# oicr-gsi/ConsensusCruncher

Measured on AMD Instinct MI355X. Metric: input reads/sec through SSCS+DCS+SC consensus, higher is better.
Workload: dtype u8

## Files before the change

consensuscruncher_amd/csrc/cc_engine.hip:

```cpp
#include <algorithm>
#include <climits>
#include <cstdint>
#include <cstdio>
#include <cstring>

#include <dlfcn.h>
#include <sched.h>

#include <chrono>

#include <hip/hip_runtime.h>
#include <atomic>
#include <map>
#include <memory>
#include <mutex>
#include <type_traits>
#include <string>
#include <unordered_set>
#include <vector>

#include "../../include/consensuscruncher_amd.h"

static std::atomic<long long> g_launches{0};
#undef hipLaunchKernelGGL
#define hipLaunchKernelGGL(kernelName, ...)                                                          \
    do {                                                                                            \
        g_launches.fetch_add(1, std::memory_order_relaxed);                                         \
        hipLaunchKernelGGLInternal((kernelName), __VA_ARGS__);                                      \
    } while (0)
#define hipMemsetAsync(...) (g_launches.fetch_add(1, std::memory_order_relaxed), ::hipMemsetAsync(__VA_ARGS__))
#define hipMemcpyAsync(...) (g_launches.fetch_add(1, std::memory_order_relaxed), ::hipMemcpyAsync(__VA_ARGS__))

enum : uint32_t {
    EB_COLLISION = 1u << 0,
    EB_DUP_QNAME = 1u << 1,
    EB_AMBIGUOUS = 1u << 2,
    EB_N_HIGHQ = 1u << 3,
    EB_BAD_BASE = 1u << 4,
    EB_SHORT = 1u << 5,
    EB_NO_QUAL = 1u << 6,
    EB_NO_CIGAR = 1u << 7,
    EB_RG = 1u << 8,
    EB_THR = 1u << 9,
    EB_TOO_LONG = 1u << 10,
    EB_KEYERROR = 1u << 12,
    EB_CHAIN = 1u << 13,
    EB_NEEDSORT = 1u << 14,
    EB_PLAN = 1u << 11,
    EB_DEEPSORT = 1u << 15,
    EB_SCANWAIT = 1u << 16,
    EB_GUARD = 1u << 17,
};

__device__ unsigned int g_guard;
__device__ __noinline__ int64_t guard_fail() {
    atomicOr(&g_guard, 1u);
    return 0;
}
#ifdef CC_DEBUG_BOUNDS
__device__ unsigned long long g_dbg_fault;
__device__ __noinline__ int64_t dbg_fail(int site, int64_t i) {
    atomicCAS(&g_dbg_fault, 0ULL, ((unsigned long long)site << 48) | ((unsigned long long)i & 0xffffffffffffULL));
    return 0;
}
__device__ __forceinline__ int64_t dbg_idx(int64_t i, int64_t n, int site) {
    return (i < 0 || i >= n) ? dbg_fail(site, i) : i;
}
#define CC_IDX(i, n, site) ((std::remove_cv_t<std::remove_reference_t<decltype(i)>>)dbg_idx((int64_t)(i), (int64_t)(n), (site)))
#elif defined(CC_NO_GUARD)
#define CC_IDX(i, n, site) (i)
#else
__device__ __forceinline__ int64_t guard_idx(int64_t i, int64_t n) {
    return (uint64_t)i < (uint64_t)n ? i : guard_fail();
}
#define CC_IDX(i, n, site) ((std::remove_cv_t<std::remove_reference_t<decltype(i)>>)guard_idx((int64_t)(i), (int64_t)(n)))
#endif
enum : int {
    DS_REC = 1, DS_QNAME = 2, DS_PAYLOAD = 3, DS_SLOT = 4, DS_PAIR = 5, DS_MEMBER = 6, DS_VOTE_REC = 7,
};

struct TagKey {
    int32_t bc, tid, pos, mtid, mpos, cigA, cigB;
    uint32_t bits;
};
struct CKey {
    int32_t bc, tidLo, posLo, tidHi, posHi, cigA, cigB;
    uint32_t strand;
    uint32_t abstlen;
    uint32_t pad[3];
};

constexpr int GRP_SMALL = 64;

struct alignas(32) RecCore {
    int32_t tid, pos, mtid, mpos, tlen, cig, bc, flag;
};

struct DevTable {
    int64_t n;
    int32_t *tid, *pos, *mtid, *mpos, *tlen, *cig, *qlen, *lseq, *bc, *rg;
    uint16_t* flag;
    uint8_t *mapq, *rflags;
    uint64_t* qn_off;
// ... 340 lines not shown
    for (int i = 4; i < nw; ++i) h = hcomb(h, w[i]);
    return hcomb(h, (uint64_t)len);
}
__device__ __forceinline__ bool qname_eq(const DevTable& T, int32_t a, int32_t b) {
    a = CC_IDX(a, T.n, DS_REC);
    b = CC_IDX(b, T.n, DS_REC);
    const uint64_t oa = T.qn_ol[a], ob = T.qn_ol[b];
    const int la = (int)(oa & 0xffffu), lb = (int)(ob & 0xffffu);
    const uint64_t* wa = reinterpret_cast<const uint64_t*>(T.qn_blob + CC_IDX(oa >> 16, T.qn_bytes + 1, DS_QNAME));
    const uint64_t* wb = reinterpret_cast<const uint64_t*>(T.qn_blob + CC_IDX(ob >> 16, T.qn_bytes + 1, DS_QNAME));
    const int nw = ((la < lb ? la : lb) + 7) >> 3;
    uint64_t d = la != lb ? 1ULL : 0ULL;
#pragma unroll
    for (int i = 0; i < 4; ++i)
        if (i < nw) d |= wa[i] ^ wb[i];
    for (int i = 4; i < nw && !d; ++i) d |= wa[i] ^ wb[i];
    return d == 0;
}

__device__ __forceinline__ int32_t readlane_i32(int32_t v, int k) { return __builtin_amdgcn_readlane(v, k); }
__device__ __forceinline__ uint64_t readlane_u64(uint64_t v, int k) {
    uint32_t lo = (uint32_t)__builtin_amdgcn_readlane((int)(uint32_t)v, k);
    uint32_t hi = (uint32_t)__builtin_amdgcn_readlane((int)(uint32_t)(v >> 32), k);
    return ((uint64_t)hi << 32) | lo;
}

__device__ __forceinline__ int64_t xcd_block() {
    const uint32_t nb = gridDim.x, b = blockIdx.x;
    const uint32_t q = nb >> 3, rem = nb & 7u, x = b & 7u;
    return (int64_t)(x * q + (x < rem ? x : rem) + (b >> 3));
}

__device__ __forceinline__ void wave_add(uint32_t v, uint32_t* dst) {
#pragma unroll
    for (int o = 32; o > 0; o >>= 1) v += __shfl_xor(v, o);
    if ((threadIdx.x & 63) == 0 && v) atomicAdd(dst, v);
}

constexpr int PSTRIPES = 64, PSTRIDE = 16;
__device__ __forceinline__ void stripe_add(uint32_t v, uint32_t* stripes) {
#pragma unroll
    for (int o = 32; o > 0; o >>= 1) v += __shfl_xor(v, o);
    const uint32_t w = blockIdx.x * (blockDim.x >> 6) + (threadIdx.x >> 6);
    if ((threadIdx.x & 63) == 0 && v) atomicAdd(stripes + PSTRIDE * (w & (PSTRIPES - 1)), v);
}

__global__ __launch_bounds__(64) void k_stripe_total(uint32_t* __restrict__ stripes, uint32_t* __restrict__ total) {
    const int t = threadIdx.x;
    uint32_t v = stripes[PSTRIDE * t];
    stripes[PSTRIDE * t] = 0u;
#pragma unroll
    for (int o = 32; o > 0; o >>= 1) v += __shfl_xor(v, o);
    if (t == 0) *total = v;
}

struct FillSet {
    static constexpr int K = 12;
    uint32_t* p[K];
    int64_t n[K];
    uint32_t v[K];
    int k;
};
__global__ __launch_bounds__(256) void k_fill(FillSet fs) {
    const int64_t stride = (int64_t)gridDim.x * blockDim.x;
    const int64_t t = (int64_t)blockIdx.x * blockDim.x + threadIdx.x;
    for (int d = 0; d < fs.k; ++d) {
        uint32_t* p = fs.p[d];
        const int64_t n = fs.n[d];
        const int64_t n4 = ((uintptr_t)p & 15u) ? 0 : n >> 2;
        const uint32_t v = fs.v[d];
        uint4* p4 = reinterpret_cast<uint4*>(p);
        for (int64_t i = t; i < n4; i += stride) p4[i] = make_uint4(v, v, v, v);
        for (int64_t i = 4 * n4 + t; i < n; i += stride) p[i] = v;
    }
}

constexpr int CNT_STRIPES = 64;
__device__ __forceinline__ unsigned long long* cnt_stripe(unsigned long long* cnt) {
    return cnt + CC_NUM_COUNTERS * (blockIdx.x & (CNT_STRIPES - 1));
}

template <int NC>
__device__ __forceinline__ void block_count(int (&v)[NC], const int (&slot)[NC], unsigned long long* cnt) {
    __shared__ int s_red[4][NC];
    const int lane = threadIdx.x & 63, wv = threadIdx.x >> 6;
#pragma unroll
    for (int c = 0; c < NC; ++c) {
        int x = v[c];
        for (int o = 32; o > 0; o >>= 1) x += __shfl_down(x, o);
        if (lane == 0) s_red[wv][c] = x;
    }
    __syncthreads();
#pragma unroll
    for (int c = 0; c < NC; ++c)
        if ((int)threadIdx.x == c) {
            int t = 0;
            for (int w = 0; w < (int)(blockDim.x >> 6); ++w) t += s_red[w][c];
            if (t) atomicAdd(&cnt_stripe(cnt)[slot[c]], (unsigned long long)t);
        }
}


struct ClassifyOut {
    uint64_t* skey;
    uint32_t* sval;
    uint8_t* badflag;
// ... 368 lines not shown
    }
    (void)qkey;
    return m == 1 ? cand : -1;
}

__device__ __forceinline__ int32_t mate_search_global(int64_t N, const uint64_t* __restrict__ rkey,
                                                      const uint64_t* __restrict__ rq, const DevTable& T,
                                                      int32_t r, int32_t mtid, int32_t mpos, uint64_t target,
                                                      uint64_t key, int64_t hint, const uint64_t* __restrict__ gq,
                                                      const int32_t* __restrict__ gend,
                                                      const uint32_t* __restrict__ boff) {
    int64_t x = 0;
    {
        int64_t hi = hint, lo = hint;
        for (int64_t step = 256;; step <<= 2) {
            lo = hi - step;
            if (lo <= 0) { lo = 0; break; }
            if (rkey[lo] < target) break;
            hi = lo;
        }
        x = lo;
        while (x < hi) {
            const int64_t mid = (x + hi) >> 1;
            if (rkey[mid] < target) x = mid + 1;
            else hi = mid;
        }
    }
    if (x + GRP_SMALL + 1 < N && rkey[x] == target && rkey[x + GRP_SMALL + 1] == target)
        return gq ? deep_find(gq, gend, boff, rq, x, key, r) : -1;
    int32_t cand = -1, m = 0, ng = 0;
    for (bool over = false; !over; x += 4) {
        uint64_t kk[4], qq[4];
#pragma unroll
        for (int u = 0; u < 4; ++u) {
            kk[u] = x + u < N ? rkey[x + u] : 0ULL;
            qq[u] = x + u < N ? rq[x + u] : 0ULL;
        }
#pragma unroll
        for (int u = 0; u < 4; ++u) {
            if (over || (x + u < N && kk[u] < target)) continue;
            if (x + u >= N || kk[u] != target) { over = true; continue; }
            if (ng > GRP_SMALL) return -1;
            ++ng;
            if (x + u != r && qq[u] == key) { cand = (int32_t)(x + u); ++m; }
        }
    }
    return m == 1 ? cand : -1;
}

__device__ __forceinline__ bool mate_record(int64_t s, int32_t sx, uint64_t key, int32_t* __restrict__ partner,
                                            int32_t* __restrict__ claimer, int32_t* __restrict__ mate_of,
                                            uint8_t* __restrict__ pflag, unsigned long long* __restrict__ ltab,
                                            uint64_t lmask, uint32_t& n_long, bool both_search,
                                            uint32_t* __restrict__ err) {
    partner[s] = sx;
    claimer[sx] = (int32_t)s;
    const int32_t s1 = (int32_t)s < sx ? (int32_t)s : sx, s2 = (int32_t)s < sx ? sx : (int32_t)s;
    mate_of[s2] = s1;
    pflag[s2] = 1;
    const bool enters = !both_search || s == s2;
    if (ltab && s2 - s1 > PD_W && enters) {
        ++n_long;
        uint64_t h = key & lmask;
        bool done = false;
        for (uint64_t i = 0; i <= lmask && !done; ++i) {
            const unsigned long long prev = atomicCAS(&ltab[h], ~0ULL, key);
            if (prev == ~0ULL) done = true;
            else if (prev == key) { atomicOr(err, EB_NEEDSORT); done = true; }
            else h = (h + 1) & lmask;
        }
        if (!done) atomicOr(err, EB_NEEDSORT);
    } else if (!ltab && s2 - s1 > PD_W && enters) {
        ++n_long;
    }
    return enters;
}

constexpr int PC_HALO = 512;
constexpr int64_t PC_SMALL_N = (int64_t)1 << 23;
template <int TILE>
__global__ __launch_bounds__(256) void k_pair_coord_tile(int64_t N, const uint64_t* __restrict__ skey,
                                                         const int32_t* __restrict__ spos,
                                                         const uint64_t* __restrict__ rkey, DevTable T,
                                                         int32_t* __restrict__ partner, int32_t* __restrict__ claimer,
                                                         int32_t* __restrict__ mate_of, uint8_t* __restrict__ pflag,
                                                         unsigned long long* __restrict__ ltab, uint64_t lmask,
                                                         uint32_t* __restrict__ long_stripes, uint32_t* __restrict__ err,
                                                         const uint64_t* __restrict__ gq, const int32_t* __restrict__ gend,
                                                         const uint32_t* __restrict__ boff,
                                                         const unsigned long long* __restrict__ dgk, uint64_t dgmask,
                                                         uint64_t* __restrict__ pkeys, uint32_t* __restrict__ pcount,
                                                         uint32_t pcap) {
    __shared__ uint64_t s_k[(TILE + PC_HALO + GRP_SMALL + 2)], s_q[(TILE + PC_HALO + GRP_SMALL + 2)];
    const int64_t t0 = xcd_block() * TILE;
    const int64_t t1 = min(N, t0 + TILE);
    const int64_t w0 = t0 > PC_HALO ? t0 - PC_HALO : 0;
    const int64_t w1 = min(N, t1 + GRP_SMALL + 2);
    const int nw = (int)(w1 - w0);
    int32_t mt[TILE / 256], mp[TILE / 256];
#pragma unroll
    for (int u = 0; u < TILE / 256; ++u) {
        const int64_t s = t0 + threadIdx.x + 256 * u;
        mt[u] = s < t1 ? T.mtid[s] : 0;
        mp[u] = s < t1 ? T.mpos[s] : 0;
    }
    for (int i = threadIdx.x; i < nw; i += blockDim.x) {
        s_k[i] = rkey[w0 + i];
        s_q[i] = skey[w0 + i];
    }
    __syncthreads();
    constexpr int PC_PER = TILE / 256;
    int32_t cand[PC_PER];
    uint64_t key[PC_PER], tgt[PC_PER];
#pragma unroll
    for (int u = 0; u < PC_PER; ++u) {
        const int64_t s = t0 + threadIdx.x + 256 * u;
        cand[u] = -1;
        key[u] = ~0ULL;
        tgt[u] = ~0ULL;
        if (s >= t1) continue;
        const int li = (int)(s - w0);
        key[u] = s_q[li];
        if (!spos) partner[s] = -1;
        if (key[u] == ~0ULL) continue;
        const int32_t r = (int32_t)s;
        const int32_t mtid = mt[u], mpos = mp[u];
        const uint64_t target = pos_key(mtid, mpos);
        tgt[u] = target;
        if (target > s_k[li]) continue;
        if (dgk) {
            const int2 dg = dg_lookup(dgk, dgmask, target);
            if (dg.x >= 0) {
                cand[u] = deep_find(gq, gend, boff, skey, dg.x, key[u], r, dg.y);
                continue;
            }
        }
        int lo = 0, hi = li;
        while (lo < hi) {
            const int mid = (lo + hi) >> 1;
            if (s_k[mid] < target) lo = mid + 1;
            else hi = mid;
        }
        if (lo == 0 && w0 > 0) {
            int x = 0;
            while (x < nw && x <= GRP_SMALL + 1 && s_k[x] == target) ++x;
            cand[u] = x > GRP_SMALL + 1 && !gq ? -1
                      : mate_search_global(N, rkey, skey, T, r, mtid, mpos, target, key[u], w0, gq, gend, boff);
        } else {
            int x = lo, ng = 0, m = 0, c = -1;
            bool deep = false;
            for (; x < nw && s_k[x] == target; ++x) {
                if (ng > GRP_SMALL) { deep = true; break; }
                ++ng;
                if (x != li && s_q[x] == key[u]) { c = (int32_t)(w0 + x); ++m; }
            }
            if (deep) c = gq ? deep_find(gq, gend, boff, skey, w0 + lo, key[u], r) : -1;
            else if (x == nw && w1 < N)
                c = mate_search_global(N, rkey, skey, T, r, mtid, mpos, target, key[u], w0 + lo, gq, gend, boff);
            else if (m != 1) c = -1;
            cand[u] = c;
        }
    }
    bool ok[PC_PER];
    {
        int la[PC_PER], lb[PC_PER];
        const uint64_t* wa[PC_PER];
        const uint64_t* wb[PC_PER];
#pragma unroll
        for (int u = 0; u < PC_PER; ++u) {
            const int32_t r = (int32_t)(t0 + threadIdx.x + 256 * u), c = cand[u] < 0 ? r : cand[u];
            const bool f = cand[u] >= 0;
            const uint64_t oa = f ? T.qn_ol[r] : 0ULL, ob = f ? T.qn_ol[c] : 0ULL;
            la[u] = (int)(oa & 0xffffu);
            lb[u] = (int)(ob & 0xffffu);
            wa[u] = reinterpret_cast<const uint64_t*>(T.qn_blob + (oa >> 16));
            wb[u] = reinterpret_cast<const uint64_t*>(T.qn_blob + (ob >> 16));
        }
#pragma unroll
        for (int u = 0; u < PC_PER; ++u) {
            const int nw8 = (la[u] + 7) >> 3;
            uint64_t d = la[u] != lb[u] ? 1ULL : 0ULL;
#pragma unroll
            for (int w = 0; w < 4; ++w)
                if (w < nw8) d |= wa[u][w] ^ wb[u][w];
            for (int w = 4; w < nw8 && !d; ++w) d |= wa[u][w] ^ wb[u][w];
            ok[u] = cand[u] >= 0 && d == 0;
        }
    }
    uint32_t nl = 0, na = 0;
    uint64_t ak[PC_PER];
#pragma unroll
    for (int u = 0; u < PC_PER; ++u) {
        ak[u] = 0;
        if (ok[u]) {
            const int32_t r = (int32_t)(t0 + threadIdx.x + 256 * u);
            const bool both = tgt[u] == rkey[r];
            const bool enters = mate_record(spos ? spos[r] : r, spos ? spos[cand[u]] : cand[u], key[u], partner,
                                            claimer, mate_of, pflag, ltab, lmask, nl, both, err);
            if (pkeys && enters) ak[na++] = key[u];
        }
    }
    stripe_add(nl, long_stripes);
    if (pkeys) {
        const int lane = threadIdx.x & 63;
        uint32_t x = na;
#pragma unroll
        for (int o = 1; o < 64; o <<= 1) {
            const uint32_t y = (uint32_t)__shfl_up((int)x, o, 64);
            if (lane >= o) x += y;
        }
        const uint32_t tot = (uint32_t)__shfl((int)x, 63, 64);
        uint32_t base = 0;
        if (lane == 63 && tot) base = atomicAdd(pcount, tot);
        base = (uint32_t)__shfl((int)base, 63, 64) + x - na;
#pragma unroll
        for (int u = 0; u < PC_PER; ++u)
            if ((uint32_t)u < na) {
                if (base + u < pcap) pkeys[base + u] = ak[u];
                else atomicOr(err, EB_PLAN);
            }
    }
}

constexpr int LP_BITS = 12, LP_BUCKETS = 1 << LP_BITS, LP_NB = 256, LP_T = 1024, LP_U = 8;
constexpr int64_t LP_MIN = 1 << 20;
constexpr int LP_SLOTS = 16384;
__device__ __forceinline__ uint32_t lp_bucket(uint64_t k) { return (uint32_t)(k >> (64 - LP_BITS)); }
__global__ __launch_bounds__(LP_T) void k_lp_hist(const uint64_t* __restrict__ keys, const uint32_t* __restrict__ count,
                                                  uint32_t cap, uint32_t* __restrict__ hist) {
    __shared__ uint32_t s_h[LP_BUCKETS];
    const uint32_t n = min(*count, cap);
    const uint32_t chunk = (n + LP_NB - 1) / LP_NB;
    const uint32_t a = blockIdx.x * chunk, b = min(n, a + chunk);
    for (int i = threadIdx.x; i < LP_BUCKETS; i += LP_T) s_h[i] = 0u;
    __syncthreads();
    for (uint32_t i0 = a + threadIdx.x; i0 < b; i0 += LP_T * LP_U) {
        uint64_t k[LP_U];
#pragma unroll
        for (int u = 0; u < LP_U; ++u) k[u] = i0 + u * LP_T < b ? keys[i0 + u * LP_T] : 0ULL;
#pragma unroll
        for (int u = 0; u < LP_U; ++u)
            if (i0 + u * LP_T < b) atomicAdd(&s_h[lp_bucket(k[u])], 1u);
    }
    __syncthreads();
    for (int i = threadIdx.x; i < LP_BUCKETS; i += LP_T) hist[(size_t)i * LP_NB + blockIdx.x] = s_h[i];
}
__global__ __launch_bounds__(LP_T) void k_lp_scatter(const uint64_t* __restrict__ keys, const uint32_t* __restrict__ count,
                                                     uint32_t cap, const uint32_t* __restrict__ off,
                                                     uint64_t* __restrict__ out) {
    __shared__ uint32_t s_o[LP_BUCKETS];
    const uint32_t n = min(*count, cap);
    const uint32_t chunk = (n + LP_NB - 1) / LP_NB;
    const uint32_t a = blockIdx.x * chunk, b = min(n, a + chunk);
    for (int i = threadIdx.x; i < LP_BUCKETS; i += LP_T) s_o[i] = off[(size_t)i * LP_NB + blockIdx.x];
// ... 146 lines not shown
        rv[x] = (uint32_t)i;
        if (!ht) return;
        atomicOr(&bloom[bloom_word(k, bmask)], (unsigned long long)bloom_bits(k));
        uint64_t slot = k & hmask;
        for (uint64_t p = 0; p <= hmask; ++p) {
            const unsigned long long prev = atomicCAS(&ht[slot], ~0ULL, k);
            if (prev == ~0ULL || prev == k) {
                if (atomicAdd(&hcnt[slot], 1u) == 2u) atomicAdd(n_multi, 1u);
                atomicMin(&hmin[slot], (uint32_t)i);
                atomicMax(&hmax[slot], (uint32_t)i);
                return;
            }
            slot = (slot + 1) & hmask;
        }
        atomicOr(err, EB_PLAN);
    }
};

__global__ __launch_bounds__(256) void k_resid_insert(const uint32_t* __restrict__ n_app, int64_t cap,
                                                      const uint64_t* __restrict__ rk, const uint32_t* __restrict__ rv,
                                                      unsigned long long* __restrict__ ht, uint64_t hmask,
                                                      unsigned long long* __restrict__ bloom, uint64_t bmask,
                                                      uint32_t* __restrict__ hcnt, uint32_t* __restrict__ hmin,
                                                      uint32_t* __restrict__ hmax, uint32_t* __restrict__ n_multi,
                                                      uint32_t* __restrict__ err) {
    const int64_t x = (int64_t)blockIdx.x * blockDim.x + threadIdx.x;
    const int64_t n = (int64_t)*n_app;
    if (x == 0 && n > cap) atomicOr(err, EB_PLAN);
    if (x >= n || x >= cap) return;
    const uint64_t k = rk[x];
    const uint32_t i = rv[x];
    atomicOr(&bloom[bloom_word(k, bmask)], (unsigned long long)bloom_bits(k));
    uint64_t slot = k & hmask;
    for (uint64_t p = 0; p <= hmask; ++p) {
        const unsigned long long prev = atomicCAS(&ht[slot], ~0ULL, k);
        if (prev == ~0ULL || prev == k) {
            if (atomicAdd(&hcnt[slot], 1u) == 2u) atomicAdd(n_multi, 1u);
            atomicMin(&hmin[slot], i);
            atomicMax(&hmax[slot], i);
            return;
        }
        slot = (slot + 1) & hmask;
    }
    atomicOr(err, EB_PLAN);
}

__global__ __launch_bounds__(256) void k_resid_pair(int64_t NR, const uint64_t* __restrict__ rk,
                                                    const uint32_t* __restrict__ rv,
                                                    const unsigned long long* __restrict__ ht, uint64_t hmask,
                                                    const uint32_t* __restrict__ hcnt, const uint32_t* __restrict__ hmin,
                                                    const uint32_t* __restrict__ hmax, int ident,
                                                    const int32_t* __restrict__ stream_rec, DevTable T,
                                                    int32_t* __restrict__ mate_of, uint8_t* __restrict__ pflag,
                                                    uint32_t* __restrict__ err, unsigned long long* __restrict__ cnt) {
    int acc[1] = {0};
    const int64_t x = (int64_t)blockIdx.x * blockDim.x + threadIdx.x;
    if (x < NR) {
        const uint64_t k = rk[x];
        const uint32_t i = rv[x];
        uint64_t slot = k & hmask;
        for (uint64_t p = 0; p <= hmask && ht[slot] != k; ++p) slot = (slot + 1) & hmask;
        const uint32_t c = hcnt[slot];
        if (c == 1u) acc[0] = 1;
        else if (c == 2u) {
            if (i == hmax[slot]) {
                const uint32_t a = hmin[slot];
                if (qname_eq(T, ident ? (int32_t)a : stream_rec[a], ident ? (int32_t)i : stream_rec[i])) {
                    mate_of[i] = (int32_t)a;
                    pflag[i] = 1;
                } else {
                    atomicOr(err, EB_COLLISION);
                }
            }
        } else {
            atomicOr(err, EB_PLAN);
        }
    }
    const int slots[1] = {CC_CNT_UNPAIRED};
    block_count<1>(acc, slots, cnt);
}

__global__ __launch_bounds__(256) void k_resid_probe(int64_t S, const uint64_t* __restrict__ skey,
                                                     const uint8_t* __restrict__ resid,
                                                     const unsigned long long* __restrict__ ht, uint64_t mask,
                                                     const unsigned long long* __restrict__ bloom, uint64_t bmask,
                                                     uint32_t* __restrict__ err) {
    const int64_t s = (int64_t)blockIdx.x * blockDim.x + threadIdx.x;
    if (s >= S) return;
    const uint64_t k = skey[s];
    if (k == ~0ULL || resid[s]) return;
    const uint64_t bb = bloom_bits(k);
    if ((bloom[bloom_word(k, bmask)] & bb) != bb) return;
    uint64_t slot = k & mask;
    for (uint64_t i = 0; i <= mask; ++i) {
        const unsigned long long h = ht[slot];
        if (h == ~0ULL) break;
        if (h == k) { atomicOr(err, EB_NEEDSORT); break; }
        slot = (slot + 1) & mask;
    }
}

__global__ __launch_bounds__(256) void k_resid_probe_sorted(int64_t S, const uint64_t* __restrict__ skey,
                                                            const uint8_t* __restrict__ resid,
                                                            const uint64_t* __restrict__ sorted, int64_t nr,
                                                            uint32_t* __restrict__ err) {
    int64_t s = (int64_t)blockIdx.x * blockDim.x + threadIdx.x;
    if (s >= S) return;
    const uint64_t k = skey[s];
    if (k == ~0ULL || resid[s]) return;
    int64_t lo = 0, hi = nr;
    while (lo < hi) {
        const int64_t mid = (lo + hi) >> 1;
        if (sorted[mid] < k) lo = mid + 1;
        else hi = mid;
    }
    if (lo < nr && sorted[lo] == k) atomicOr(err, EB_NEEDSORT);
}


__global__ __launch_bounds__(256) void k_pair_keys(int64_t P, PairView V, DevTable T, uint64_t seed,
                                                   uint64_t* __restrict__ chash, uint64_t* __restrict__ thash,
                                                   uint32_t* __restrict__ tval, int4* __restrict__ ptag,
                                                   uint64_t* __restrict__ rec_hash, uint2* __restrict__ bigE,
                                                   int4* __restrict__ rec_tag) {
    const int64_t p = (int64_t)blockIdx.x * blockDim.x + threadIdx.x;
    if (p >= P) return;
    const int32_t a = V.rec1[p], b = V.rec2[p];
    const uint32_t run = pair_run(V, (int32_t)p);
    const RecCore A = T.core[CC_IDX(a, T.n, DS_REC)], B = T.core[CC_IDX(b, T.n, DS_REC)];
    if (bigE) bigE[p] = make_uint2((A.flag & CORE_DEEP) ? 1u : 0u, (B.flag & CORE_DEEP) ? 1u : 0u);
// ... 268 lines not shown
        const uint32_t rg7 = rg < 0 ? 0x7fu : (rg >= 126 ? 0x7eu : (uint32_t)rg);
        const uint32_t w = ((uint32_t)f & 0xfffu) | (mq << 12) | ((rfl & 7u) << 20) | (rg7 << 24);
        RecCore c;
        c.tid = tid; c.pos = pos; c.mtid = mt; c.mpos = mp;
        c.tlen = tl; c.cig = cg; c.bc = bc; c.flag = f | (deep ? CORE_DEEP : 0);
        const bool last = li + 1 >= hi || (s_k[li + 1] >> 32) != (k >> 32);
        if (tid >= 0 && tid < T.ntid && last) T.ext[tid] = pos < 0 ? 0 : pos;
        T.rkey[r] = k;
        T.meta[r] = make_uint4((uint32_t)(po >> 4), (uint32_t)tl, lq, w);
        T.core[r] = c;
        T.rdeep[r] = deep ? 1 : 0;
        T.qn_ol[r] = (qo << 16) | qlen;
        const uint64_t qd = h & T.qdig_mask;
        T.qdig[r] = qd;
        if (CLS) {
            bool listed = false;
            const uint64_t key = classify_key((int32_t)r, dc.stream_region[r], f, (uint8_t)rfl, qd, dc.region_run, T,
                                              dc.delim_filter, dc.badread, dc.scoped, dc.seed, dc.use_dig, acc, listed);
            if (dc.o.badflag) dc.o.badflag[r] = listed ? 1 : 0;
            dc.o.skey[r] = key;
            dc.o.mate_of[r] = -1;
            dc.o.pflag[r] = 0;
            if (dc.o.claimer) dc.o.claimer[r] = -1;
            if (dc.rec_e) dc.rec_e[r] = -1;
        }
    }
    if (CLS) {
        if (r == 0) {
            const uint32_t eb = *T.ebits;
            if (eb) atomicOr(dc.err, eb);
        }
        classify_count(acc, dc.cnt);
    }
    const uint64_t m = __ballot(dstart);
    if (m) {
        const int lane = t & 63, ld = __ffsll((unsigned long long)m) - 1;
        uint32_t base = 0;
        if (lane == ld) base = atomicAdd(ndeep, (uint32_t)__popcll(m));
        base = (uint32_t)__shfl((int)base, ld, 64);
        if (dstart) {
            const uint32_t o = base + (uint32_t)__popcll(m & ((1ULL << lane) - 1ULL));
            if ((int64_t)o < dcap) dlist[o] = (int32_t)r;
        }
    }
}

template <bool BYREC>
__global__ __launch_bounds__(GT) void k_group_rank(int64_t N, const uint64_t* __restrict__ rkey,
                                                   const int32_t* __restrict__ rec_e, const uint64_t* __restrict__ rhash,
                                                   const uint32_t* __restrict__ tile_pre,
                                                   uint64_t* __restrict__ rs_key, uint32_t* __restrict__ rs_val,
                                                   int32_t* __restrict__ rs_rec, PairView V, const int4* __restrict__ rec_tag,
                                                   DevTable T, uint8_t* __restrict__ segf, uint32_t* __restrict__ validf,
                                                   uint4* __restrict__ mem_meta, uint32_t* __restrict__ err) {
    __shared__ uint64_t s_k[GS], s_h[GS];
    __shared__ int32_t s_e[GS];
    __shared__ int4 s_t[BYREC ? GS : 1];
    __shared__ int2 s_m[BYREC ? GS : 1];
    __shared__ uint32_t s_hd[GW];
    __shared__ uint32_t s_c[GT / 64];
    const int64_t b0 = xcd_block() * GT;
    const int t = threadIdx.x;
    const int nt = (int)(N - b0 < GT ? N - b0 : GT);
    const uint32_t base = tile_pre[b0 / GT];
    int lo, hi;
    tile_range(N, b0, nt, lo, hi);
    for (int i = t; i < GS; i += GT) {
        if (i < lo || i >= hi) continue;
        const int64_t rr = b0 - GH + i;
        s_k[i] = rkey[rr];
        s_e[i] = rec_e[rr];
        s_h[i] = rhash[rr];
        if constexpr (BYREC) {
            s_t[i] = rec_tag[rr];
            s_m[i] = make_int2(T.mtid[rr], T.mpos[rr]);
        }
    }
    __syncthreads();
    tile_heads(s_k, lo, hi, s_hd);
    __syncthreads();
    const int32_t r = (int32_t)(b0 + t);
    const int li = t + GH;
    int a = 0, z = 0;
    bool sm = false;
    if (t < nt && s_e[li] >= 0) {
        tile_span(s_hd, li, a, z);
        sm = z - a <= GRP_SMALL;
    }
    const uint64_t bm = __ballot(sm);
    const int lane = t & 63;
    if (lane == 0) s_c[t >> 6] = (uint32_t)__popcll(bm);
    __syncthreads();
    if (!sm) return;
    const int fo = BYREC ? 0 : (int)T.flag[r];
    const int32_t omt = BYREC ? 0 : T.mtid[r], omp = BYREC ? 0 : T.mpos[r];
    const uint4 om = mem_meta ? T.meta[CC_IDX(r, T.n, DS_MEMBER)] : make_uint4(0u, 0u, 0u, 0u);
    uint32_t cpv = base + (uint32_t)__popcll(bm & ((1ULL << lane) - 1ULL));
    for (int w = 0; w < (t >> 6); ++w) cpv += s_c[w];
    const int32_t e = s_e[li];
    const uint64_t h = s_h[li];
    uint32_t before = 0, rank = 0;
    int32_t pe = -1, pj = 0;
    uint64_t ph = 0;
    for (int j = a; j < z; ++j) {
        const int32_t ej = s_e[j];
        if (ej < 0) continue;
        const uint64_t hj = s_h[j];
        before += j < li ? 1u : 0u;
        if (hj < h || (hj == h && ej < e)) {
            ++rank;
            if (pe < 0 || hj > ph || (hj == ph && ej > pe)) { pe = ej; ph = hj; pj = j; }
        }
    }
    const uint32_t o = CC_IDX(cpv - before + rank, N, DS_SLOT);
    bool start = pe < 0 || ph != h;
    if (!start) {
        bool same;
        if constexpr (BYREC) {
            const int4 x = s_t[li], y = s_t[pj];
            const int2 mx = s_m[li], my = s_m[pj];
            same = x.x == y.x && x.y == y.y && x.z == y.z && x.w == y.w && mx.x == my.x && mx.y == my.y;
        } else {
            const int32_t rp = (int32_t)(b0 - GH + pj);
            const int4 pt = V.tag[e >> 1], pq = V.tag[pe >> 1];
            const int fp = T.flag[rp];
            same = pt.x == pq.x && pt.y == pq.y && pt.z == pq.z && pt.w == pq.w && omt == T.mtid[rp] &&
                   omp == T.mpos[rp] && ((fo >> 4) & 1) == ((fp >> 4) & 1) && which_read(fo) == which_read(fp);
        }
        if (!same) {
            atomicOr(err, EB_COLLISION);
            start = true;
        }
    }
    const bool valid = start || ((e >> 1) != (pe >> 1));
    if (start) rs_key[o] = h;
    rs_val[o] = (uint32_t)e;
    rs_rec[o] = r;
    segf[o] = start ? 1 : 0;
    validf[o] = valid ? 1u : 0u;
    if (mem_meta) {
        uint4 m = om;
        m.w |= (valid ? 1u : 0u) << 23;
        mem_meta[o] = m;
    }
}

__global__ __launch_bounds__(256) void k_big_keys(int64_t R, const uint32_t* __restrict__ bigE,
                                                  const uint32_t* __restrict__ bx, const uint64_t* __restrict__ rhash,
                                                  PairView V, const uint32_t* __restrict__ gid, int gbits, int kb,
                                                  uint64_t* __restrict__ bkey, uint32_t* __restrict__ bval) {
    int64_t e = (int64_t)blockIdx.x * blockDim.x + threadIdx.x;
    if (e >= R || !bigE[e]) return;
    const int32_t r = (e & 1) ? V.rec2[e >> 1] : V.rec1[e >> 1];
    const uint64_t h = rhash[r];
    bkey[bx[e]] = gid ? (((uint64_t)gid[r] << (kb - gbits)) | (h >> (64 - kb + gbits))) : h;
    bval[bx[e]] = (uint32_t)e;
}

constexpr int DF_T = 512, DF_SLOTS = 1024, DF_FAMS = 512, DF_SORT = 8192, DF_ST = 512;
constexpr unsigned long long DF_EMPTY = ~0ULL;

__device__ __forceinline__ uint32_t df_slot0(uint64_t h) { return (uint32_t)(h ^ (h >> 31)) & (DF_SLOTS - 1); }
__device__ __forceinline__ int df_find(const unsigned long long* s_key, uint64_t h) {
    uint32_t s = df_slot0(h);
    for (int p = 0; p < DF_SLOTS; ++p) {
        const unsigned long long k = s_key[s];
        if (k == h) return (int)s;
        if (k == DF_EMPTY) return -1;
        s = (s + 1) & (DF_SLOTS - 1);
    }
    return -1;
}
__device__ __forceinline__ uint64_t shfl64(uint64_t v, int src) {
    const uint32_t lo = (uint32_t)__shfl((int)(uint32_t)v, src, 64);
    const uint32_t hi = (uint32_t)__shfl((int)(uint32_t)(v >> 32), src, 64);
    return ((uint64_t)hi << 32) | lo;
}
__device__ __forceinline__ TagKey shfl_tag(const TagKey& t, int src) {
    TagKey o;
    const int32_t* m = reinterpret_cast<const int32_t*>(&t);
    int32_t* p = reinterpret_cast<int32_t*>(&o);
#pragma unroll
    for (int k = 0; k < 8; ++k) p[k] = __shfl(m[k], src, 64);
    return o;
}
__device__ __forceinline__ uint32_t wave_sort(uint32_t v, int lane) {
#pragma unroll
    for (int k = 2; k <= 64; k <<= 1)
#pragma unroll
        for (int j = k >> 1; j > 0; j >>= 1) {
            const uint32_t u = (uint32_t)__shfl_xor((int)v, j, 64);
            v = (((lane & j) == 0) == ((lane & k) == 0)) ? min(v, u) : max(v, u);
        }
    return v;
}

__global__ __launch_bounds__(256) void k_deep_count(const uint32_t* __restrict__ ndeep, const int32_t* __restrict__ dlist,
// ... 415 lines not shown
                    const uint32_t i = (uint32_t)((h + k) * DF_ST + t);
                    v[k] = i < p2 ? A[i] : 0u;
                    lo[k] = (i & ~(2 * w - 1)) + ((i & w) ? 0u : w);
                }
                for (uint32_t sp = w >> 1; sp > 0; sp >>= 1) {
#pragma unroll
                    for (int k = 0; k < SE / 2; ++k) {
                        const uint32_t i = (uint32_t)((h + k) * DF_ST + t);
                        const uint32_t pm = A[lo[k] + sp - 1];
                        if ((i & w) ? (pm <= v[k]) : (pm < v[k])) lo[k] += sp;
                    }
                }
#pragma unroll
                for (int k = 0; k < SE / 2; ++k) {
                    const uint32_t i = (uint32_t)((h + k) * DF_ST + t);
                    if (i >= p2) continue;
                    const uint32_t pm = A[lo[k]];
                    if ((i & w) ? (pm <= v[k]) : (pm < v[k])) lo[k] += 1;
                    const uint32_t st = i & ~(2 * w - 1), other = st + ((i & w) ? 0u : w);
                    B[st + (i & (w - 1)) + (lo[k] - other)] = v[k];
                }
            }
            __syncthreads();
            uint32_t* tmp = A; A = B; B = tmp;
        }
        for (int h = 0; h < SE; h += SE / 2) {
            uint32_t v[SE / 2];
            int32_t r[SE / 2];
#pragma unroll
            for (int k = 0; k < SE / 2; ++k) {
                const uint32_t i = (uint32_t)((h + k) * DF_ST + t);
                v[k] = i < m ? A[i] : 0u;
                r[k] = i < m ? CC_IDX((v[k] & 1u) ? V.rec2[v[k] >> 1] : V.rec1[v[k] >> 1], T.n, DS_REC) : 0;
            }
#pragma unroll
            for (int k = 0; k < SE / 2; ++k) {
                const uint32_t i = (uint32_t)((h + k) * DF_ST + t);
                if (i < m) deep_put(out, V, T, d.z + (int64_t)i, v[k], r[k], i == 0, i == 0 || (v[k] >> 1) != (A[i - 1] >> 1), err);
            }
        }
    }
}

__global__ __launch_bounds__(256) void k_fam_build(int64_t F, int64_t R, int64_t n_known, int one_region,
                                                   const int32_t* __restrict__ fam_beg,
                                                   const int32_t* __restrict__ fam_drop,
                                                   const uint32_t* __restrict__ rs_val, const uint64_t* __restrict__ rs_key,
                                                   const int32_t* __restrict__ pr_region, const uint64_t* __restrict__ rhash,
                                                   const int32_t* __restrict__ mem_rec, int32_t* __restrict__ fam_end,
                                                   int32_t* __restrict__ fam_n, int32_t* __restrict__ fam_first,
                                                   int32_t* __restrict__ fam_region, uint64_t* __restrict__ fam_hash,
                                                   uint8_t* __restrict__ cflag, int32_t* __restrict__ cfam,
                                                   int32_t* __restrict__ fam_o, PairView V, DevTable T,
                                                   TagKey* __restrict__ fam_tag, int32_t* __restrict__ fam_rec) {
    int64_t f = (int64_t)blockIdx.x * blockDim.x + threadIdx.x;
    if (f < F) {
        fam_o[f] = 0x7f7f7f7f;
        int32_t b = CC_IDX(fam_beg[f], R, DS_SLOT);
        int32_t e = (f + 1 < F) ? fam_beg[f + 1] : (int32_t)R;
        if (e < b || e > R) e = b + (int32_t)guard_fail() + 1;
        fam_end[f] = e;
        fam_n[f] = e - b - fam_drop[f];
        uint32_t fe = rs_val[b];
        fam_first[f] = (int32_t)fe;
        fam_region[f] = one_region ? 0 : pr_region[fe >> 1];
        fam_hash[f] = rhash && b >= n_known ? rhash[CC_IDX(mem_rec[b], T.n, DS_REC)] : rs_key[b];
        cflag[fe] = 1;
        cfam[fe] = (int32_t)f;
        if (fam_tag) {
            const int32_t r0 = mem_rec[b];
            fam_tag[f] = tag_of_rec(T, r0, V.tag[fe >> 1]);
            fam_rec[f] = r0;
        }
    }
}

__global__ __launch_bounds__(256) void k_fam_tags(int64_t F, const int32_t* __restrict__ fam_first,
                                                  const int32_t* __restrict__ fam_beg, const int32_t* __restrict__ mem_rec,
                                                  PairView V, DevTable T, TagKey* __restrict__ fam_tag,
                                                  int32_t* __restrict__ fam_rec) {
    const int64_t f = (int64_t)blockIdx.x * blockDim.x + threadIdx.x;
    if (f < F) {
        const int32_t r0 = mem_rec[fam_beg[f]];
        fam_tag[f] = tag_of_rec(T, r0, V.tag[fam_first[f] >> 1]);
        fam_rec[f] = r0;
    }
}

__global__ __launch_bounds__(256) void k_csn_keys(int64_t F, const int32_t* __restrict__ fam_by_k,
                                                  const int32_t* __restrict__ fam_first, const uint64_t* __restrict__ chash,
                                                  uint64_t* __restrict__ ekey, uint32_t* __restrict__ eval) {
    int64_t k = (int64_t)blockIdx.x * blockDim.x + threadIdx.x;
    if (k >= F) return;
    int32_t f = fam_by_k[k];
    ekey[k] = chash[fam_first[f] >> 1];
    eval[k] = (uint32_t)k;
}

__global__ __launch_bounds__(256) void k_csn_mark(int64_t F, const uint64_t* __restrict__ es_key,
                                                  const uint32_t* __restrict__ es_val, const int32_t* __restrict__ fam_by_k,
                                                  const int32_t* __restrict__ fam_first, PairView V, DevTable T,
                                                  uint32_t* __restrict__ segf, uint32_t* __restrict__ err) {
    int64_t j = (int64_t)blockIdx.x * blockDim.x + threadIdx.x;
    if (j >= F) return;
    bool start = (j == 0) || es_key[j - 1] != es_key[j];
    if (!start) {
        int32_t pa = fam_first[fam_by_k[es_val[j]]] >> 1, pb = fam_first[fam_by_k[es_val[j - 1]]] >> 1;
        if (!ckey_eq(ckey_of_pair(T, V, pa), ckey_of_pair(T, V, pb))) {
            atomicOr(err, EB_COLLISION);
            start = true;
        }
    }
    segf[j] = start;
}

__global__ __launch_bounds__(256) void k_overlap_keyerror(int64_t E, const int32_t* __restrict__ ent_f,
                                                          const int32_t* __restrict__ fam_beg,
                                                          const int32_t* __restrict__ fam_end,
                                                          const int32_t* __restrict__ fam_region,
                                                          const uint32_t* __restrict__ rs_val,
                                                          const int32_t* __restrict__ pr_region,
                                                          uint32_t* __restrict__ err) {
    const int64_t q = (int64_t)blockIdx.x * blockDim.x + threadIdx.x;
    if (q >= E) return;
    const int32_t fa = ent_f[2 * q], fb = ent_f[2 * q + 1];
    if (fb < 0) return;
    const int32_t rc = max(fam_region[fa], fam_region[fb]);
// ... 17 lines not shown
    if (f >= F) return;
    const int32_t gd = fam_del[f];
    if (gd == NEVER_DELETED) return;
    const int32_t j = fam_end[f] - 1;
    if (j >= fam_beg[f] && pr_region[rs_val[j] >> 1] > gd) atomicOr(err, EB_KEYERROR);
}
__global__ __launch_bounds__(256) void k_dcs_deleted(int64_t F, const int32_t* __restrict__ fam_o,
                                                     const int32_t* __restrict__ fam_region, int64_t Q,
                                                     const int32_t* __restrict__ dec, int32_t* __restrict__ fam_del) {
    const int64_t f = (int64_t)blockIdx.x * blockDim.x + threadIdx.x;
    if (f >= F) return;
    const int32_t q = fam_o[f];
    fam_del[f] = (q >= 0 && (int64_t)q < Q && (dec[q] == 0 || dec[q] == 1)) ? fam_region[f] : NEVER_DELETED;
}

__global__ __launch_bounds__(256) void k_csn_entries(int64_t F, const uint32_t* __restrict__ segf,
                                                     const uint32_t* __restrict__ es_val,
                                                     const int32_t* __restrict__ fam_by_k,
                                                     const int32_t* __restrict__ fam_region, int per_region,
                                                     uint8_t* __restrict__ emark, int32_t* __restrict__ e1k,
                                                     unsigned long long* __restrict__ cnt) {
    int64_t j = (int64_t)blockIdx.x * blockDim.x + threadIdx.x;
    if (j >= F || !segf[j]) return;
    int64_t m = 1;
    while (j + m < F && !segf[j + m]) ++m;
    unsigned long long orphans = 0;
    auto reg = [&](int64_t i) { return fam_region[fam_by_k[es_val[j + i]]]; };
    for (int64_t i = 0; i < m;) {
        const uint32_t k0 = es_val[j + i];
        const int32_t r0 = reg(i);
        emark[k0] = 1;
        if (i + 1 >= m || (per_region && reg(i + 1) != r0)) {
            e1k[k0] = -1;
            ++i;
            continue;
        }
        e1k[k0] = (int32_t)es_val[j + i + 1];
        const int32_t rc = reg(i + 1);
        i += 2;
        while (i < m && reg(i) == rc) { ++orphans; ++i; }
    }
    if (orphans) atomicAdd(&cnt_stripe(cnt)[CC_CNT_ORPHAN_TAGS], orphans);
}

constexpr int64_t CT = 1024;
constexpr int CW = 2 * GRP_SMALL;
constexpr int CSLOTS = 2048;
static_assert(CSLOTS >= CT + CW + 1, "the tile table holds every start of the tile and its window");
__global__ __launch_bounds__(256) void k_csn_fast(int64_t F, const int32_t* __restrict__ pair_by_k,
                                                  const uint64_t* __restrict__ chash,
                                                  const uint32_t* __restrict__ bigE,
                                                  unsigned long long* __restrict__ ht_key, uint64_t mask,
                                                  uint8_t* __restrict__ emark, int32_t* __restrict__ e1k,
                                                  uint32_t* __restrict__ shared) {
    __shared__ int32_t s_p[CT + CW + 2];
    __shared__ unsigned long long s_tab[CSLOTS];
    const int t = threadIdx.x;
    const int64_t t0 = (int64_t)blockIdx.x * CT, t1 = min(F, t0 + CT);
    const int64_t w0 = max((int64_t)0, t0 - CW - 1), w1 = min(F, t1 + 1);
    for (int64_t k = w0 + t; k < w1; k += blockDim.x) s_p[k - w0] = pair_by_k[k];
    for (int i = t; i < CSLOTS; i += blockDim.x) s_tab[i] = ~0ULL;
    __syncthreads();
    bool sh = false;
    for (int64_t k = (w0 == 0 ? 0 : w0 + 1) + t; k < t1; k += blockDim.x) {
        const int32_t p = s_p[k - w0];
        const bool start = (k == 0) || s_p[k - 1 - w0] != p;
        if (k >= t0) {
            emark[k] = start ? 1 : 0;
            if (start) e1k[k] = (k + 1 < F && s_p[k + 1 - w0] == p) ? (int32_t)(k + 1) : -1;
        }
        if (!start) continue;
        const unsigned long long h = chash[p];
        if (bigE && !bigE[2 * p] && !bigE[2 * p + 1]) {
            uint32_t slot = (uint32_t)(h >> 13) & (CSLOTS - 1);
            bool done = false;
            for (int i = 0; i < CSLOTS && !done; ++i) {
                const unsigned long long prev = atomicCAS(&s_tab[slot], ~0ULL, h);
                if (prev == ~0ULL) done = true;
                else if (prev == h) { sh = true; done = true; }
                else slot = (slot + 1) & (CSLOTS - 1);
            }
            if (!done) sh = true;
        } else if (k >= t0) {
            uint64_t slot = h & mask;
            bool done = false;
            for (uint64_t i = 0; i <= mask && !done; ++i) {
                const unsigned long long prev = atomicCAS(&ht_key[slot], ~0ULL, h);
                if (prev == ~0ULL) done = true;
                else if (prev == h) { sh = true; done = true; }
                else slot = (slot + 1) & mask;
            }
            if (!done) sh = true;
        }
    }
    if (sh) *shared = 1u;
}


__global__ __launch_bounds__(256) void k_emit_keys(int64_t E, const uint8_t* __restrict__ has2,
                                                   const int32_t* __restrict__ ent_f,
                                                   const int32_t* __restrict__ fam_region, uint64_t* __restrict__ key,
                                                   uint32_t* __restrict__ val) {
    const int64_t r = (int64_t)blockIdx.x * blockDim.x + threadIdx.x;
    if (r >= E) return;
    uint64_t k = ~0ULL;
    if (has2[r]) {
        const int32_t rc = max(fam_region[ent_f[2 * r]], fam_region[ent_f[2 * r + 1]]);
        k = ((uint64_t)((uint32_t)rc ^ 0x80000000u) << 32) | (uint64_t)r;
    }
    key[r] = k;
    val[r] = (uint32_t)r;
}
__global__ __launch_bounds__(256) void k_emit_rank(int64_t E2, const uint32_t* __restrict__ sval,
                                                   uint32_t* __restrict__ hx) {
    const int64_t j = (int64_t)blockIdx.x * blockDim.x + threadIdx.x;
    if (j < E2) hx[sval[j]] = (uint32_t)j;
}

__global__ __launch_bounds__(256) void k_sscs_emit(int64_t E, const int32_t* __restrict__ ent_f,
                                                   const int32_t* __restrict__ ent_pair,
                                                   const uint8_t* __restrict__ has2, const uint32_t* __restrict__ hx,
                                                   const int32_t* __restrict__ fam_n, const int32_t* __restrict__ fam_beg,
                                                   const int32_t* __restrict__ fam_end,
                                                   const int32_t* __restrict__ mem_rec, int32_t* __restrict__ emit_fam,
                                                   int32_t* __restrict__ emit_n, int32_t* __restrict__ emit_rec,
                                                   uint8_t* __restrict__ needv, int2* __restrict__ emit_span,
                                                   PairView V, DevTable T, int32_t* __restrict__ ent_ckey) {
    int64_t r = (int64_t)blockIdx.x * blockDim.x + threadIdx.x;
    if (r >= E) return;
    const uint8_t two = has2[r];
    const uint32_t x = hx[r];
    const int2 ff = *reinterpret_cast<const int2*>(ent_f + 2 * r);
    const int32_t pr = ent_pair[r];
    if (!two) return;
    const uint32_t o = 2 * x;
    const int32_t f2[2] = {ff.x, ff.y};
    int32_t b2[2], n2[2], e2[2], m2[2];
#pragma unroll
    for (int s = 0; s < 2; ++s) { b2[s] = fam_beg[f2[s]]; n2[s] = fam_n[f2[s]]; e2[s] = fam_end[f2[s]]; }
#pragma unroll
    for (int s = 0; s < 2; ++s) m2[s] = mem_rec[b2[s]];
    const CKey c = ckey_of_pair(T, V, pr);
#pragma unroll
    for (int s = 0; s < 2; ++s) {
        emit_fam[o + s] = f2[s];
        emit_n[o + s] = n2[s];
        emit_rec[o + s] = m2[s];
        needv[o + s] = n2[s] >= 2 ? 1 : 0;
// ... 1343 lines not shown
            *reinterpret_cast<uint2*>(out_seq + w * (int64_t)(qstride >> 1) + (i0 >> 1)) =
                make_uint2((code[0] << 4) | code[1], (code[2] << 4) | code[3]);
        }
        if (c == 0) {
            const int fa = (int)(ma.w & 0xfffu), fb = (int)(mb.w & 0xfffu);
            int32_t mapq = (int32_t)((ma.w >> 12) & 0xffu), tlen = (int32_t)ma.y, flag = fa, rg;
            const int32_t ra = TA.rg[a], rb = TBx.rg[b];
            if (sc) {
                rg = ra;
                if ((ma.w >> 20) & CC_RF_RG_UNSUPPORTED) eb |= EB_RG;
            } else {
                if (fa == fb) flag = fa;
                else if (fa == 99 || fb == 99) flag = 99;
                else if (fa == 83 || fb == 83) flag = 83;
                else if (fa == 147 || fb == 147) flag = 147;
                else if (fa == 163 || fb == 163) flag = 163;
                rg = (ra >= 0 && rb >= 0) ? ra : -1;
                if (((ma.w | mb.w) >> 20) & CC_RF_RG_UNSUPPORTED) eb |= EB_RG;
            }
            out_meta[5 * w + 0] = L;
            out_meta[5 * w + 1] = mapq;
            out_meta[5 * w + 2] = tlen;
            out_meta[5 * w + 3] = flag;
            out_meta[5 * w + 4] = rg;
        }
    }
#pragma unroll
    for (int o = 32; o > 0; o >>= 1) eb |= __shfl_xor(eb, o);
    if (lane == 0 && eb) atomicOr(err, eb);
}

__global__ __launch_bounds__(256) void k_ckey_out(int64_t n, const int32_t* __restrict__ pairs, PairView V,
                                                  DevTable T, int32_t* __restrict__ out9) {
    int64_t i = (int64_t)blockIdx.x * blockDim.x + threadIdx.x;
    if (i >= n) return;
    int32_t p = pairs[i];
    int32_t* o = out9 + 9 * i;
    if (p < 0) {
        for (int k = 0; k < 9; ++k) o[k] = -1;
        return;
    }
    const CKey c = ckey_of_pair(T, V, p);
    o[0] = c.bc; o[1] = c.tidLo; o[2] = c.posLo; o[3] = c.tidHi; o[4] = c.posHi;
    o[5] = c.cigA; o[6] = c.cigB; o[7] = (int32_t)(c.strand & 3u); o[8] = (int32_t)c.abstlen;
}

__global__ __launch_bounds__(256) void k_q_pairs(int64_t Q, const int32_t* __restrict__ ent_pair,
                                                 int32_t* __restrict__ out) {
    int64_t q = (int64_t)blockIdx.x * blockDim.x + threadIdx.x;
    if (q < Q) out[q] = ent_pair[q >> 1];
}


constexpr int SCAN_T = 256, SCAN_I = 16, SCAN_TILE = SCAN_T * SCAN_I;

template <bool MAX>
__device__ __forceinline__ uint32_t sop(uint32_t a, uint32_t b) { return MAX ? (a > b ? a : b) : a + b; }

__device__ __forceinline__ void scan_load_tile(const uint32_t* __restrict__ in, int64_t n, int64_t base,
                                               uint32_t* s_tile, uint32_t v[SCAN_I]) {
    const int tid = threadIdx.x;
    if (base + SCAN_TILE <= n) {
#pragma unroll
        for (int j = 0; j < SCAN_I / 4; ++j) {
            const int o = (j * SCAN_T + tid) * 4;
            reinterpret_cast<uint4*>(s_tile)[o >> 2] = *reinterpret_cast<const uint4*>(in + base + o);
        }
    } else {
        for (int o = tid; o < SCAN_TILE; o += SCAN_T) s_tile[o] = base + o < n ? in[base + o] : 0u;
    }
    __syncthreads();
#pragma unroll
    for (int j = 0; j < SCAN_I / 4; ++j) {
        const int jj = (j + (tid >> 1)) & 3;
        const uint4 q = reinterpret_cast<const uint4*>(s_tile)[tid * 4 + jj];
        v[4 * jj + 0] = q.x; v[4 * jj + 1] = q.y; v[4 * jj + 2] = q.z; v[4 * jj + 3] = q.w;
    }
}

template <bool MAX>
__device__ __forceinline__ uint32_t block_scan_excl(uint32_t x, uint32_t* s_w, uint32_t* tot) {
    const int tid = threadIdx.x, lane = tid & 63, w = tid >> 6;
    uint32_t inc = x;
#pragma unroll
    for (int o = 1; o < 64; o <<= 1) {
        const uint32_t y = __shfl_up(inc, o, 64);
        if (lane >= o) inc = sop<MAX>(inc, y);
    }
    if (lane == 63) s_w[w] = inc;
    __syncthreads();
    uint32_t pre = 0, all = 0;
#pragma unroll
    for (int j = 0; j < SCAN_T / 64; ++j) {
        if (j < w) pre = sop<MAX>(pre, s_w[j]);
        all = sop<MAX>(all, s_w[j]);
    }
    *tot = all;
    uint32_t ex = __shfl_up(inc, 1, 64);
    if (lane == 0) ex = 0;
    return sop<MAX>(pre, ex);
}

__device__ __forceinline__ uint32_t byte_sum(uint32_t w) { return (w * 0x01010101u) >> 24; }

template <bool MAX, class TIn>
__global__ __launch_bounds__(SCAN_T) void k_scan_reduce(const TIn* __restrict__ in, int64_t n,
                                                        uint32_t* __restrict__ part) {
// ... 120 lines not shown
    const int32_t *t_rec, *p_rec, *dec;
    int32_t* vslot;
    int4* vpair;
    struct Ld { int32_t t, p, d; };
    __device__ Ld ld1(int64_t i, uint32_t f) const { return f ? Ld{t_rec[i], p_rec[i], dec[i]} : Ld{0, 0, 0}; }
    __device__ void ld2(Ld&, uint32_t) const {}
    __device__ void st(int64_t i, uint32_t x, uint32_t f, const Ld& l) const {
        vslot[i] = f ? (int32_t)x : -1;
        if (f) vpair[x] = make_int4(l.t, l.p, l.d, (int32_t)i);
    }
    __device__ void operator()(int64_t i, uint32_t x, uint32_t f) const {
        Ld l = ld1(i, f);
        st(i, x, f, l);
    }
};
struct EmitList {
    static constexpr bool kPlain = false;
    int32_t *vslot, *list;
    __device__ void operator()(int64_t i, uint32_t x, uint32_t f) const {
        vslot[i] = f ? (int32_t)x : -1;
        if (f) list[x] = (int32_t)i;
    }
};
struct EmitEntries {
    static constexpr bool kPlain = false, kStaged = true;
    const int32_t *e1k, *fam_by_k, *pair_by_k;
    int32_t *ent_f, *ent_pair, *fam_o;
    uint8_t* has2;
    struct Ld { int32_t f0, k1, pr; };
    __device__ Ld ld1(int64_t k, uint32_t f) const {
        return f ? Ld{fam_by_k[k], e1k[k], pair_by_k[k]} : Ld{-1, -1, -1};
    }
    __device__ void ld2(Ld& l, uint32_t f) const { l.k1 = f && l.k1 >= 0 ? fam_by_k[l.k1] : -1; }
    __device__ void st(int64_t, uint32_t r, uint32_t f, const Ld& l) const {
        if (!f) return;
        const int32_t f0 = l.f0, f1 = l.k1;
        ent_f[2 * r] = f0;
        ent_f[2 * r + 1] = f1;
        has2[r] = f1 >= 0 ? 1 : 0;
        ent_pair[r] = l.pr;
        fam_o[f0] = (int32_t)(2 * r);
        if (f1 >= 0) fam_o[f1] = (int32_t)(2 * r + 1);
    }
    __device__ void operator()(int64_t k, uint32_t r, uint32_t f) const {
        Ld l = ld1(k, f);
        ld2(l, f);
        st(k, r, f, l);
    }
};

template <bool MAX, class Emit, class TIn>
__global__ __launch_bounds__(SCAN_T) void k_scan_down(const TIn* __restrict__ in, int64_t n,
                                                      const uint32_t* __restrict__ part,
                                                      uint32_t* __restrict__ total, Emit em) {
    __shared__ uint32_t s_tile[SCAN_TILE];
    __shared__ uint32_t s_w[SCAN_T / 64];
    __shared__ uint32_t s_pre[SCAN_T / 64];
    const int64_t base = (int64_t)blockIdx.x * SCAN_TILE;
    const int tid = threadIdx.x;
    uint32_t pre = 0;
    for (uint32_t i = tid; i < blockIdx.x; i += SCAN_T) pre = sop<MAX>(pre, part[i]);
#pragma unroll
    for (int o = 32; o > 0; o >>= 1) pre = sop<MAX>(pre, __shfl_xor(pre, o, 64));
    if ((tid & 63) == 0) s_pre[tid >> 6] = pre;
    uint32_t v[SCAN_I];
    if constexpr (sizeof(TIn) == 1) {
        if (base + SCAN_TILE <= n) {
            const uint4 q = *reinterpret_cast<const uint4*>(in + base + tid * SCAN_I);
            const uint32_t w[4] = {q.x, q.y, q.z, q.w};
#pragma unroll
            for (int k = 0; k < SCAN_I; ++k) v[k] = (w[k >> 2] >> (8 * (k & 3))) & 0xffu;
        } else {
#pragma unroll
            for (int k = 0; k < SCAN_I; ++k) {
                const int64_t i = base + tid * SCAN_I + k;
                v[k] = i < n ? (uint32_t)in[i] : 0u;
            }
        }
        __syncthreads();
    } else {
        scan_load_tile(in, n, base, s_tile, v);
    }
    pre = 0;
#pragma unroll
    for (int j = 0; j < SCAN_T / 64; ++j) pre = sop<MAX>(pre, s_pre[j]);
    uint32_t t = 0;
#pragma unroll
    for (int k = 0; k < SCAN_I; ++k) t = sop<MAX>(t, v[k]);
    uint32_t all;
    uint32_t run = sop<MAX>(pre, block_scan_excl<MAX>(t, s_w, &all));
    if (blockIdx.x == gridDim.x - 1 && tid == 0) *total = sop<MAX>(pre, all);
#pragma unroll
    for (int k = 0; k < SCAN_I; ++k) {
        const uint32_t x = v[k];
        if (MAX) { run = sop<MAX>(run, x); v[k] = run; }
        else { v[k] = run; run += x; }
    }
#pragma unroll
    for (int j = 0; j < SCAN_I / 4; ++j) {
        const int jj = (j + (tid >> 1)) & 3;
        reinterpret_cast<uint4*>(s_tile)[tid * 4 + jj] = make_uint4(v[4 * jj], v[4 * jj + 1], v[4 * jj + 2], v[4 * jj + 3]);
    }
    __syncthreads();
    if (base + SCAN_TILE <= n) {
#pragma unroll
        for (int j = 0; j < SCAN_I / 4; ++j) {
            const int o = (j * SCAN_T + tid) * 4;
            const uint4 x = reinterpret_cast<const uint4*>(s_tile)[o >> 2];
            if constexpr (Emit::kPlain) {
                *reinterpret_cast<uint4*>(em.out + base + o) = x;
            } else if constexpr (sizeof(TIn) == 1 && is_staged<Emit>::value) {
                continue;
            } else if constexpr (sizeof(TIn) == 1) {
                const uint32_t f = *reinterpret_cast<const uint32_t*>(in + base + o);
                em(base + o, x.x, f & 0xffu);
                em(base + o + 1, x.y, (f >> 8) & 0xffu);
                em(base + o + 2, x.z, (f >> 16) & 0xffu);
                em(base + o + 3, x.w, f >> 24);
            } else {
                const uint4 f = *reinterpret_cast<const uint4*>(in + base + o);
                em(base + o, x.x, f.x);
                em(base + o + 1, x.y, f.y);
                em(base + o + 2, x.z, f.z);
                em(base + o + 3, x.w, f.w);
            }
        }
        if constexpr (!Emit::kPlain && sizeof(TIn) == 1 && is_staged<Emit>::value) {
            typename Emit::Ld ld[SCAN_I];
            uint32_t fx[SCAN_I], xx[SCAN_I];
#pragma unroll
            for (int j = 0; j < SCAN_I / 4; ++j) {
                const int o = (j * SCAN_T + tid) * 4;
                const uint4 x = reinterpret_cast<const uint4*>(s_tile)[o >> 2];
                const uint32_t f = *reinterpret_cast<const uint32_t*>(in + base + o);
                xx[4 * j] = x.x; xx[4 * j + 1] = x.y; xx[4 * j + 2] = x.z; xx[4 * j + 3] = x.w;
#pragma unroll
                for (int k = 0; k < 4; ++k) fx[4 * j + k] = (f >> (8 * k)) & 0xffu;
            }
#pragma unroll
            for (int e = 0; e < SCAN_I; ++e) ld[e] = em.ld1(base + ((e >> 2) * SCAN_T + tid) * 4 + (e & 3), fx[e]);
#pragma unroll
            for (int e = 0; e < SCAN_I; ++e) em.ld2(ld[e], fx[e]);
#pragma unroll
            for (int e = 0; e < SCAN_I; ++e) em.st(base + ((e >> 2) * SCAN_T + tid) * 4 + (e & 3), xx[e], fx[e], ld[e]);
// ... 269 lines not shown
}

namespace {

struct DevBuf {
    void* p = nullptr;
    size_t bytes = 0;
    size_t used = 0;
};

struct Group {
    int32_t table = -1;
    int64_t S = 0, P = 0, R = 0, F = 0, E = 0, Q = 0, NV = 0;
    uint64_t seed = 0;
    int scoped = 0, delim_filter = 0, badread = 0;
    uint64_t ht_mask = 0;
    bool csn_fast = false;
    bool stripes_pending = false;
    bool no_deep_fam = false;
    int coord_sorted = 0;
    bool force_sort = false;
    int ident = 0;
    bool local_groups = false;
    int64_t counters[CC_NUM_COUNTERS] = {0};
    std::map<std::string, DevBuf> buf;
    std::map<std::string, int64_t> plan;
    std::map<std::string, int> slot;
    std::map<std::string, bool> planned;
    bool fast = false;
    bool members_built = false;
    int64_t n_deepg = 0;
    bool fam_tags_built = false;
    bool overlap = false;
    int32_t n_regions = 1;
    std::vector<std::string> verify;
    std::vector<int32_t> swap_host;
    double thr_cutoff = -1.0;
};

struct DeferredCheck {
    Group* g = nullptr;
    int32_t gid = -1;
    int slot = 0;
    bool counters = false;
    bool bad_listed = false;
    std::vector<std::pair<int, int64_t>> expect;
};
constexpr int DEFER_SLOTS = 64;
constexpr size_t DEFER_SLOT_BYTES = 12288;

constexpr int CC_E_PLAN = -100;
constexpr int CC_E_NEEDSORT = -101;
constexpr int CC_E_DEEPSORT = -102;
constexpr int CC_E_SCANWAIT = -103;
constexpr int PLAN_SLOTS = 64;

}

struct BgzfEnc;

struct cc_ctx {
    int device = 0;
    hipStream_t stream = nullptr;
    std::string err;
    std::map<int32_t, DevTable> tables;
    std::map<int32_t, std::vector<void*>> table_allocs;
    std::map<int32_t, std::unique_ptr<Group>> groups;
    int32_t next_id = 1;
    DevBuf tmp;
    DevBuf sort_buf;
    unsigned long long* scan_st = nullptr;
    uint32_t* scan_ticket = nullptr;
    int64_t scan_cap = 0;
    uint32_t scan_epoch = 0;
    uint32_t scan_spin_max = 1u << 22;
    bool scan_two = false;
    std::unordered_set<int32_t> full_qhash;
    int64_t scan_retries = 0;
    int64_t guard_reruns = 0;
    uint32_t* d_err = nullptr;
    unsigned long long* d_cnt = nullptr;
    void* h_pinned = nullptr;
    std::atomic<bool> profiling{false};
    std::unordered_set<std::string> prof_only;
    struct Prof { double ms = 0; int64_t n = 0; };
    std::map<std::string, Prof> prof;
    std::vector<std::pair<std::string, std::pair<hipEvent_t, hipEvent_t>>> pending;
    std::vector<hipEvent_t> event_pool;
    std::unique_ptr<Group> scratch;
    bool defer = false;
    std::vector<DeferredCheck> deferred;
    uint8_t* h_defer = nullptr;
    uint8_t* d_defer = nullptr;
    BgzfEnc* bgzf = nullptr;
    std::mutex bgzf_mu;
};

namespace {

#define HIPCHK(x)                                                                               \
    do {                                                                                        \
        hipError_t e_ = (x);                                                                    \
        if (e_ != hipSuccess) {                                                                 \
            ctx->err = std::string("HIP error ") + hipGetErrorString(e_) + " at " #x;           \
            return CC_E_HIP;                                                                    \
        }                                                                                       \
    } while (0)

#define RC(x)                     \
    do {                          \
        int rc_ = (x);            \
        if (rc_) return rc_;      \
    } while (0)

inline unsigned nblk(int64_t n, int b = 256) { return (unsigned)((n + b - 1) / b); }

struct Fills {
    cc_ctx* ctx;
    FillSet fs{};
    int64_t maxw = 0;
    explicit Fills(cc_ctx* c) : ctx(c) { fs.k = 0; }
    int add(void* p, size_t bytes, uint32_t word) {
        if (!p || bytes < 4) return 0;
        if (fs.k == FillSet::K) { int rc = launch(); if (rc) return rc; }
        fs.p[fs.k] = (uint32_t*)p;
        fs.n[fs.k] = (int64_t)(bytes / 4);
        fs.v[fs.k] = word;
        maxw = std::max<int64_t>(maxw, (int64_t)(bytes / 4));
        ++fs.k;
        return 0;
    }
// ... 32 lines not shown
            return nullptr;
        }
        ctx->tmp.bytes = nb;
    }
    return ctx->tmp.p;
}

struct ProfScope {
    cc_ctx* ctx;
    const char* name;
    hipEvent_t a = nullptr, b = nullptr;
    static hipEvent_t take(cc_ctx* ctx) {
        hipEvent_t e = nullptr;
        if (!ctx->event_pool.empty()) {
            e = ctx->event_pool.back();
            ctx->event_pool.pop_back();
        } else {
            (void)hipEventCreate(&e);
        }
        return e;
    }
    ProfScope(cc_ctx* c, const char* n) : ctx(c), name(n) {
        if (ctx->profiling && !ctx->prof_only.empty() && !ctx->prof_only.count(n)) name = nullptr;
        if (ctx->profiling && name) {
            a = take(ctx);
            b = take(ctx);
            (void)hipEventRecord(a, ctx->stream);
        }
    }
    ~ProfScope() {
        if (ctx->profiling && name) {
            (void)hipEventRecord(b, ctx->stream);
            ctx->pending.push_back({name, {a, b}});
        }
    }
};

void flush_prof(cc_ctx* ctx) {
    if (ctx->pending.empty()) return;
    (void)hipStreamSynchronize(ctx->stream);
    for (auto& p : ctx->pending) {
        float ms = 0;
        (void)hipEventElapsedTime(&ms, p.second.first, p.second.second);
        auto& pr = ctx->prof[p.first];
        pr.ms += ms;
        pr.n += 1;
        ctx->event_pool.push_back(p.second.first);
        ctx->event_pool.push_back(p.second.second);
    }
    ctx->pending.clear();
}

template <bool MAX, class Emit, class TIn>
int scan_launch(cc_ctx* ctx, const TIn* in, int64_t n, uint32_t* d_tot, const char* name, Emit em);

int sort_pairs(cc_ctx* ctx, const uint64_t* kin, uint64_t* kout, const uint32_t* vin, uint32_t* vout, int64_t n,
               const char* name, unsigned begin_bit = 0, unsigned end_bit = 64) {
    if (n <= 0) return 0;
    if (n > (int64_t)UINT32_MAX - 1) { ctx->err = "sort: more than 2^32 - 2 pairs"; return CC_E_UNSUPPORTED; }
    const int passes = end_bit > begin_bit ? (int)((end_bit - begin_bit + 7) / 8) : 0;
    const int64_t nt = (n + RS_TILE - 1) / RS_TILE;
    const size_t need = (size_t)n * 12 + 2 * sizeof(uint32_t) * (size_t)RS_BINS * (size_t)nt + 256;
    if (ctx->sort_buf.bytes < need) {
        if (ctx->sort_buf.p) {
            HIPCHK(hipStreamSynchronize(ctx->stream));
            (void)hipFree(ctx->sort_buf.p);
        }
        ctx->sort_buf.p = nullptr;
        ctx->sort_buf.bytes = 0;
        const size_t nb = need + need / 4;
        HIPCHK(hipMalloc(&ctx->sort_buf.p, nb));
        ctx->sort_buf.bytes = nb;
    }
    uint8_t* sb = (uint8_t*)ctx->sort_buf.p;
    uint64_t* tk = (uint64_t*)sb;
    uint32_t* tv = (uint32_t*)(sb + (size_t)n * 8);
    uint32_t* hist = (uint32_t*)(sb + (((size_t)n * 12 + 127) & ~(size_t)127));
    uint32_t* off = hist + (size_t)RS_BINS * nt;
    uint32_t* tot = (uint32_t*)ctx->d_err + 14;
    ProfScope ps(ctx, name);
    if (passes == 0) {
        HIPCHK(hipMemcpyAsync(kout, kin, sizeof(uint64_t) * n, hipMemcpyDeviceToDevice, ctx->stream));
        HIPCHK(hipMemcpyAsync(vout, vin, sizeof(uint32_t) * n, hipMemcpyDeviceToDevice, ctx->stream));
        return 0;
    }
    const uint64_t* sk = kin;
    const uint32_t* sv = vin;
    for (int p = 0; p < passes; ++p) {
        const int shift = (int)begin_bit + 8 * p;
        uint64_t* dk = ((passes - p) & 1) ? kout : tk;
        uint32_t* dv = ((passes - p) & 1) ? vout : tv;
        hipLaunchKernelGGL(k_rs_hist, dim3((unsigned)nt), dim3(RS_T), 0, ctx->stream, sk, n, shift, hist, nt);
        RC(scan_launch<false>(ctx, (const uint32_t*)hist, (int64_t)RS_BINS * nt, tot, "sort_scan", ScanStore{off}));
        hipLaunchKernelGGL(k_rs_scatter, dim3((unsigned)nt), dim3(RS_T), 0, ctx->stream, sk, sv, n, shift,
                           (const uint32_t*)off, nt, dk, dv);
        sk = dk;
        sv = dv;
    }
    return 0;
}

constexpr int64_t SCAN_ONE_MAX = 64;
template <bool MAX, class Emit, class TIn>
int scan_launch(cc_ctx* ctx, const TIn* in, int64_t n, uint32_t* d_tot, const char* name, Emit em) {
    const int64_t nb = (n + SCAN_TILE - 1) / SCAN_TILE;
    uintptr_t al = (uintptr_t)in;
    if constexpr (Emit::kPlain) al |= (uintptr_t)em.out;
    if (al & 15u) { ctx->err = "scan operands must be 16-B aligned"; return CC_E_INVALID; }
    const char* force = getenv("CC_SCAN1");
    const bool one = !ctx->scan_two && (force ? force[0] == '1' : nb <= SCAN_ONE_MAX);
    if (one && nb > 0) {
        if (nb > ctx->scan_cap) {
            const int64_t cap = std::max<int64_t>(nb, 1 << 14);
            if (ctx->scan_st) {
                HIPCHK(hipStreamSynchronize(ctx->stream));
                (void)hipFree(ctx->scan_st);
            }
            ctx->scan_st = nullptr;
            ctx->scan_cap = 0;
            HIPCHK(hipMalloc((void**)&ctx->scan_st, sizeof(unsigned long long) * cap + 64));
            HIPCHK(hipMemsetAsync(ctx->scan_st, 0, sizeof(unsigned long long) * cap + 64, ctx->stream));
            ctx->scan_ticket = reinterpret_cast<uint32_t*>(ctx->scan_st + cap);
            ctx->scan_cap = cap;
            ctx->scan_epoch = 0;
        }
        if (++ctx->scan_epoch >= (1u << 30)) {
            HIPCHK(hipMemsetAsync(ctx->scan_st, 0, sizeof(unsigned long long) * ctx->scan_cap, ctx->stream));
            ctx->scan_epoch = 1;
        }
        const ScanLB lb{ctx->scan_st, ctx->scan_ticket, ctx->scan_epoch, ctx->d_err, ctx->scan_spin_max};
        ProfScope ps(ctx, name);
        hipLaunchKernelGGL((k_scan_one<MAX, Emit, TIn>), dim3((unsigned)nb), dim3(SCAN_T), 0, ctx->stream, in, n, nb,
                           d_tot, em, lb);
        return 0;
    }
    int rc = 0;
    uint32_t* part = (uint32_t*)tmp_storage(ctx, (size_t)nb * 4 + 64, &rc);
    if (!part) return rc;
    ProfScope ps(ctx, name);
    hipLaunchKernelGGL((k_scan_reduce<MAX, TIn>), dim3((unsigned)nb), dim3(SCAN_T), 0, ctx->stream, in, n, part);
    hipLaunchKernelGGL((k_scan_down<MAX, Emit, TIn>), dim3((unsigned)nb), dim3(SCAN_T), 0, ctx->stream, in, n, part, d_tot, em);
    return 0;
}



hipError_t stream_wait(cc_ctx* ctx) {
    const auto t0 = std::chrono::steady_clock::now();
    for (uint32_t i = 0;; ++i) {
        const hipError_t e = hipStreamQuery(ctx->stream);
        if (e != hipErrorNotReady) return e;
        if ((i & 63u) == 63u && std::chrono::steady_clock::now() - t0 > std::chrono::microseconds(200)) sched_yield();
    }
}

int dbg_fault(cc_ctx* ctx) {
#ifdef CC_DEBUG_BOUNDS
    unsigned long long f = 0;
    HIPCHK(hipMemcpyFromSymbol(&f, HIP_SYMBOL(g_dbg_fault), sizeof(f), 0, hipMemcpyDeviceToHost));
    if (f) {
        const unsigned long long zero = 0;
        HIPCHK(hipMemcpyToSymbol(HIP_SYMBOL(g_dbg_fault), &zero, sizeof(zero), 0, hipMemcpyHostToDevice));
        static const char* names[] = {"?", "record index", "qname offset", "payload offset", "ranked slot", "pair",
                                      "member record", "vote record"};
        const int site = (int)(f >> 48);
        char buf[160];
        snprintf(buf, sizeof buf, "device bounds check failed: %s %lld out of range (debug build)",
                 names[site >= 0 && site < 8 ? site : 0], (long long)(int64_t)(f & 0xffffffffffffULL));
        ctx->err = buf;
        return CC_E_INVALID;
    }
#else
    (void)ctx;
#endif
    return 0;
}

int Fills::launch() {
    if (fs.k == 0) return 0;
    const unsigned blocks = std::min<unsigned>(nblk((maxw + 3) / 4), 2048u);
    hipLaunchKernelGGL(k_fill, dim3(blocks), dim3(256), 0, ctx->stream, fs);
    fs.k = 0;
    maxw = 0;
    return hipGetLastError() == hipSuccess ? 0 : CC_E_HIP;
}

uint32_t* plan_slot(cc_ctx* ctx, Group& g, const char* name, int* rc) {
    uint32_t* dtot = gbuf<uint32_t>(ctx, g, "plan_totals", PLAN_SLOTS, rc);
    if (*rc) return nullptr;
    auto it = g.slot.find(name);
    const int s = it != g.slot.end() ? it->second : (int)g.slot.size();
    if (s >= PLAN_SLOTS) { ctx->err = "too many planned totals"; *rc = CC_E_INVALID; return nullptr; }
    g.slot[name] = s;
    return dtot + s;
}

uint32_t* plan_stripes(cc_ctx* ctx, Group& g, uint32_t* slot, int* rc) {
    const bool fresh = !g.buf.count("plan_stripes") || !g.buf["plan_stripes"].p;
    uint32_t* st = gbuf<uint32_t>(ctx, g, "plan_stripes", (int64_t)PLAN_SLOTS * PSTRIPES * PSTRIDE, rc);
    if (*rc) return nullptr;
    if (fresh && hipMemsetAsync(st, 0, sizeof(uint32_t) * PLAN_SLOTS * PSTRIPES * PSTRIDE, ctx->stream) != hipSuccess) {
        *rc = CC_E_HIP;
        return nullptr;
    }
    return st + (slot - (uint32_t*)g.buf["plan_totals"].p) * (int64_t)PSTRIPES * PSTRIDE;
}

int planned_total(cc_ctx* ctx, Group& g, const char* name, uint32_t* d_tot, int64_t* total) {
    if (g.fast && g.plan.count(name)) {
        *total = g.plan[name];
        g.verify.push_back(name);
        return 0;
    }
    uint32_t* h = (uint32_t*)ctx->h_pinned;
    HIPCHK(hipMemcpyAsync(h, d_tot, 4, hipMemcpyDeviceToHost, ctx->stream));
    HIPCHK(stream_wait(ctx));
    *total = (int64_t)h[0];
    g.plan[name] = *total;
    return 0;
}

template <class TIn>
int scan_total(cc_ctx* ctx, Group& g, const TIn* in, uint32_t* out, int64_t n, int64_t* total,
               const char* name) {
    if (n <= 0) { *total = 0; return 0; }
    int rc = 0;
    uint32_t* d_tot = plan_slot(ctx, g, name, &rc);
    if (rc) return rc;
    RC(scan_launch<false>(ctx, in, n, d_tot, name, ScanStore{out}));
    return planned_total(ctx, g, name, d_tot, total);
}

template <class Emit, class TIn>
int scan_emit(cc_ctx* ctx, Group& g, const TIn* in, int64_t n, int64_t* total, const char* name, Emit em) {
    if (n <= 0) { *total = 0; return 0; }
    int rc = 0;
    uint32_t* d_tot = plan_slot(ctx, g, name, &rc);
    if (rc) return rc;
    RC(scan_launch<false>(ctx, in, n, d_tot, name, em));
    return planned_total(ctx, g, name, d_tot, total);
}

int finish_pass(cc_ctx* ctx, Group& g, uint32_t* bits, bool counters, bool* plan_ok) {
    if (ctx->defer && g.fast && ctx->h_defer && ctx->deferred.size() < (size_t)DEFER_SLOTS) {
        DeferredCheck d;
        d.g = &g;
        for (auto& kv : ctx->groups)
            if (kv.second.get() == &g) d.gid = kv.first;
        d.slot = (int)ctx->deferred.size();
        d.counters = counters;
        d.bad_listed = g.counters[CC_CNT_BAD_LISTED] > 0;
        uint8_t* dh = ctx->d_defer + (size_t)d.slot * DEFER_SLOT_BYTES;
        const bool totals = !g.verify.empty();
        hipLaunchKernelGGL(k_defer_pack, dim3(1), dim3(256), 0, ctx->stream, (const uint32_t*)ctx->d_err,
                           counters ? (const unsigned long long*)ctx->d_cnt : nullptr,
                           totals ? (const uint32_t*)g.buf["plan_totals"].p : nullptr, PLAN_SLOTS,
                           g.stripes_pending ? (const uint32_t*)g.buf["plan_stripes"].p : nullptr, dh);
        g.stripes_pending = false;
        if (totals)
            for (const auto& nm : g.verify) d.expect.push_back({g.slot[nm], g.plan[nm]});
        g.verify.clear();
        ctx->deferred.push_back(std::move(d));
        *bits = 0;
        *plan_ok = true;
        return 0;
    }
    uint8_t* h = (uint8_t*)ctx->h_pinned;
    hipLaunchKernelGGL(k_guard_fold, dim3(1), dim3(64), 0, ctx->stream, ctx->d_err);
    HIPCHK(hipMemcpyAsync(h + 16, ctx->d_err, 4, hipMemcpyDeviceToHost, ctx->stream));
    if (counters)
        HIPCHK(hipMemcpyAsync(h + 1024, ctx->d_cnt, sizeof(unsigned long long) * CC_NUM_COUNTERS * CNT_STRIPES,
                              hipMemcpyDeviceToHost,
                              ctx->stream));
    if (g.stripes_pending) {
        hipLaunchKernelGGL(k_stripe_fold, dim3(1), dim3(64), 0, ctx->stream, (const uint32_t*)g.buf["plan_stripes"].p,
                           (uint32_t*)g.buf["plan_totals"].p, PLAN_SLOTS);
        g.stripes_pending = false;
    }
    if (!g.verify.empty())
        HIPCHK(hipMemcpyAsync(h + 256, g.buf["plan_totals"].p, 4 * PLAN_SLOTS, hipMemcpyDeviceToHost, ctx->stream));
    HIPCHK(stream_wait(ctx));
    RC(dbg_fault(ctx));
    *bits = *(uint32_t*)(h + 16);
    if ((*bits & EB_GUARD) && g.fast) ++ctx->guard_reruns;
    const bool cap_over = (*bits & EB_PLAN) != 0 || (g.fast && (*bits & EB_GUARD) != 0);
    *bits &= g.fast ? ~(EB_PLAN | EB_GUARD) : ~EB_PLAN;
    if (counters)
        for (int i = 0; i < CC_NUM_COUNTERS; ++i) {
            int64_t t = 0;
            for (int k = 0; k < CNT_STRIPES; ++k) t += (int64_t)((unsigned long long*)(h + 1024))[CC_NUM_COUNTERS * k + i];
            g.counters[i] = t;
        }
    *plan_ok = !cap_over;
    for (const auto& nm : g.verify)
        if ((int64_t)((uint32_t*)(h + 256))[g.slot[nm]] != g.plan[nm]) *plan_ok = false;
    g.verify.clear();
    return 0;
}

template <typename Pass>
int run_planned(cc_ctx* ctx, Group& g, const char* stage, Pass pass) {
    int rc = CC_E_PLAN;
    if (g.planned[stage]) {
        g.fast = true;
        g.verify.clear();
        rc = pass();
        g.fast = false;
    }
    if (rc == CC_E_PLAN) {
        g.verify.clear();
        rc = pass();
    }
    if (rc == CC_E_SCANWAIT && !ctx->scan_two) {
        ++ctx->scan_retries;
        if (getenv("CC_SCAN_SPIN_MAX")) fprintf(stderr, "[cc] %s: look-back scan bound hit, pass re-run (%lld)\n", stage,
                                                (long long)ctx->scan_retries);
        ctx->scan_two = true;
        g.verify.clear();
        rc = pass();
        ctx->scan_two = false;
    }
    if (rc == CC_E_SCANWAIT) rc = CC_E_INVALID;
    g.planned[stage] = rc == 0;
    return rc;
}

int read_err(cc_ctx* ctx, uint32_t* bits) {
    uint32_t* h = (uint32_t*)ctx->h_pinned + 4;
    hipLaunchKernelGGL(k_guard_fold, dim3(1), dim3(64), 0, ctx->stream, ctx->d_err);
    HIPCHK(hipMemcpyAsync(h, ctx->d_err, 4, hipMemcpyDeviceToHost, ctx->stream));
    HIPCHK(stream_wait(ctx));
    *bits = *h;
    return dbg_fault(ctx);
}

int err_code(cc_ctx* ctx, uint32_t bits) {
    if (!bits) return 0;
    if (bits & EB_COLLISION) { ctx->err = "64-bit key hash collision (retry with another seed)"; return CC_E_COLLISION; }
    if (bits & EB_KEYERROR) { ctx->err = "KeyError: read_dict[tag] already deleted (consensus_helper.py:490 with overlapping bed regions, or DCS_maker.py:258 with duplex keys that are not mutual)"; return CC_E_KEYERROR; }
    if (bits & EB_AMBIGUOUS) { ctx->err = "duplex keys are not mutual or span regions; reference outcome is order-dependent"; return CC_E_AMBIGUOUS; }
    if (bits & EB_N_HIGHQ) { ctx->err = "IndexError: N base with quality >= 30 in a family of size >= 2 (SSCS_maker.py:129)"; return CC_E_N_HIGHQ; }
    if (bits & EB_SHORT) { ctx->err = "IndexError: read shorter than the consensus length"; return CC_E_SHORT_READ; }
    if (bits & EB_BAD_BASE) { ctx->err = "ValueError: base outside ACGTN in a voted family (SSCS_maker.py:122)"; return CC_E_BAD_BASE; }
    if (bits & EB_NO_QUAL) { ctx->err = "TypeError: read without base qualities in a vote"; return CC_E_NO_QUAL; }
    if (bits & EB_NO_CIGAR) { ctx->err = "TypeError: infer_query_length() is None (no cigar)"; return CC_E_NO_CIGAR; }
    if (bits & EB_RG) { ctx->err = "RG tag of a non-string type"; return CC_E_UNSUPPORTED; }
    if (bits & EB_THR) { ctx->err = "cutoff table too short"; return CC_E_INVALID; }
    if (bits & EB_CHAIN) { ctx->err = "a chain of duplex partners longer than the engine follows"; return CC_E_UNSUPPORTED; }
    if (bits & EB_SCANWAIT) { ctx->err = "scan look-back wait bound exceeded"; return CC_E_SCANWAIT; }
    if (bits & EB_TOO_LONG) { ctx->err = "record too long for the 16-bit length fields or payload > 64 GiB"; return CC_E_UNSUPPORTED; }
    if (bits & EB_GUARD) { ctx->err = "a guarded index was outside its array (no load was made from it)"; return CC_E_INVALID; }
    ctx->err = "unknown device error";
    return CC_E_INVALID;
}

template <typename T>
int upload(cc_ctx* ctx, std::vector<void*>& allocs, T** dst, const T* src, int64_t count) {
    size_t bytes = (size_t)std::max<int64_t>(count, 1) * sizeof(T);
    HIPCHK(hipMalloc((void**)dst, bytes));
    allocs.push_back(*dst);
    if (count > 0) HIPCHK(hipMemcpyAsync(*dst, src, (size_t)count * sizeof(T), hipMemcpyHostToDevice, ctx->stream));
    return 0;
}

#define GB(T, name, count) gbuf<T>(ctx, g, name, count, &brc); if (brc) return brc

int deleted_late(cc_ctx* ctx, Group& g, const int32_t* fdel) {
    if (g.F <= 0) return 0;
    hipLaunchKernelGGL(k_deleted_late, dim3(nblk(g.F)), dim3(256), 0, ctx->stream, g.F, fdel,
                       (const int32_t*)g.buf["fam_beg"].p, (const int32_t*)g.buf["fam_end"].p,
                       (const uint32_t*)g.buf["rs_val"].p, (const int32_t*)g.buf["pr_region"].p, ctx->d_err);
    return 0;
}

int build_ht(cc_ctx* ctx, Group& g) {
    int brc = 0;
    uint64_t size = 1024;
    while (size < (uint64_t)(2 * g.F)) size <<= 1;
    g.ht_mask = size - 1;
    unsigned long long* key = GB(unsigned long long, "ht_key", (int64_t)size);
    int32_t* val = GB(int32_t, "ht_val", (int64_t)size);
    HIPCHK(hipMemsetAsync(key, 0xff, sizeof(unsigned long long) * size, ctx->stream));
    if (g.F > 0) {
        ProfScope ps(ctx, "k_ht_insert");
        hipLaunchKernelGGL(k_ht_insert, dim3(nblk(g.F)), dim3(256), 0, ctx->stream, g.F,
                           (const uint64_t*)g.buf["fam_hash"].p, key, val, g.ht_mask);
    }
    return 0;
}

int upload_swap(cc_ctx* ctx, Group& g, int32_t* d_swap, const int32_t* bc_swap, int32_t n_bc) {
    if (n_bc <= 0) return 0;
    if ((int32_t)g.swap_host.size() == n_bc && !memcmp(g.swap_host.data(), bc_swap, sizeof(int32_t) * n_bc)) return 0;
    g.swap_host.assign(bc_swap, bc_swap + n_bc);
    HIPCHK(hipMemcpyAsync(d_swap, bc_swap, sizeof(int32_t) * n_bc, hipMemcpyHostToDevice, ctx->stream));
    return 0;
}

PairView pair_view(Group& g) {
    return PairView{(const int32_t*)g.buf["pr_rec1"].p, (const int32_t*)g.buf["pr_rec2"].p,
                    (const int32_t*)g.buf["pr_region"].p, (const int32_t*)g.buf["region_run"].p, g.scoped,
                    (const int4*)g.buf["pr_tag"].p};
// ... 206 lines not shown
            g.counters[CC_CNT_COUNTER] = g.S - g.counters[CC_CNT_FOREIGN] - g.counters[CC_CNT_UNMAPPED];
        }
        if (!d.counters && d.bad_listed != (g.counters[CC_CNT_BAD_LISTED] > 0)) ok = false;
    }
    ctx->deferred.clear();
    if (!ok) {
        ctx->err = "a deferred pass did not hold its plan or met an error: replay the calls with deferral off";
        return CC_E_REPLAY;
    }
    return 0;
}

int cc_debug_poison(cc_ctx* ctx, int32_t group_id, const char* name, int64_t bytes, int32_t value) {
    if (!ctx || !name || !ctx->groups.count(group_id) || bytes < 0) return CC_E_INVALID;
    Group& g = *ctx->groups[group_id];
    if (!g.buf.count(name)) { ctx->err = std::string("no buffer named ") + name; return CC_E_INVALID; }
    DevBuf& b = g.buf[name];
    const size_t used = b.used;
    int brc = 0;
    uint8_t* p = gbuf<uint8_t>(ctx, g, name, std::max<int64_t>(bytes, (int64_t)b.bytes), &brc);
    if (brc) return brc;
    b.used = used;
    HIPCHK(hipMemsetAsync(p, value & 0xff, b.bytes, ctx->stream));
    HIPCHK(hipStreamSynchronize(ctx->stream));
    return 0;
}

int cc_debug_skew_plan(cc_ctx* ctx, int32_t group_id, const char* name, int64_t delta) {
    if (!ctx || !name || !ctx->groups.count(group_id)) return CC_E_INVALID;
    Group& g = *ctx->groups[group_id];
    if (!g.plan.count(name)) { ctx->err = std::string("no planned total named ") + name; return CC_E_INVALID; }
    g.plan[name] += delta;
    return 0;
}

int cc_synchronize(cc_ctx* ctx) {
    if (!ctx) return CC_E_INVALID;
    HIPCHK(hipStreamSynchronize(ctx->stream));
    flush_prof(ctx);
    return dbg_fault(ctx);
}

int cc_debug_build(void) {
#ifdef CC_DEBUG_BOUNDS
    return 1;
#else
    return 0;
#endif
}

int64_t cc_launch_count(void) { return g_launches.load(std::memory_order_relaxed); }

int64_t cc_guard_reruns(cc_ctx* ctx) { return ctx ? ctx->guard_reruns : CC_E_INVALID; }

}
namespace {
int derive_table(cc_ctx* ctx, DevTable& T) {
    if (T.n <= 0) return 0;
    HIPCHK(hipMemsetAsync(T.ndeep, 0, 16, ctx->stream));
    ProfScope ps(ctx, "k_derive");
    hipLaunchKernelGGL(k_derive<false>, dim3(nblk(T.n, GT)), dim3(GT), 0, ctx->stream, T, T.dlist, T.ndeep,
                       T.n / DEEP_MIN + 2, DeriveCls{});
    HIPCHK(hipGetLastError());
    return 0;
}
int flush_derive(cc_ctx* ctx, int32_t id) {
    auto it = ctx->tables.find(id);
    if (it == ctx->tables.end() || !it->second.derive_pending) return 0;
    it->second.derive_pending = false;
    return derive_table(ctx, it->second);
}
}
extern "C" {

int cc_table_derive(cc_ctx* ctx, int32_t table_id) {
    if (!ctx || !ctx->tables.count(table_id)) return CC_E_INVALID;
    if (ctx->tables[table_id].host_layout) return 0;
    if (getenv("CC_DERIVE_SEPARATE")) return derive_table(ctx, ctx->tables[table_id]);
    ctx->tables[table_id].derive_pending = true;
    return 0;
}

int cc_table_upload(cc_ctx* ctx, const cc_records* r, int32_t max_len, int32_t* table_id) {
    if (!ctx || !r || !table_id) return CC_E_INVALID;
    HIPCHK(hipSetDevice(ctx->device));
    int32_t id = ctx->next_id++;
    std::vector<void*>& al = ctx->table_allocs[id];
    DevTable T;
    T.n = r->n;
    T.max_len = max_len;
    RC(upload(ctx, al, &T.tid, r->tid, r->n));
    RC(upload(ctx, al, &T.pos, r->pos, r->n));
    RC(upload(ctx, al, &T.mtid, r->mtid, r->n));
    RC(upload(ctx, al, &T.mpos, r->mpos, r->n));
    RC(upload(ctx, al, &T.tlen, r->tlen, r->n));
    RC(upload(ctx, al, &T.flag, r->flag, r->n));
    RC(upload(ctx, al, &T.mapq, r->mapq, r->n));
    RC(upload(ctx, al, &T.cig, r->cigar_id, r->n));
    RC(upload(ctx, al, &T.qlen, r->qlen, r->n));
    RC(upload(ctx, al, &T.lseq, r->lseq, r->n));
    RC(upload(ctx, al, &T.bc, r->bc_id, r->n));
    RC(upload(ctx, al, &T.rg, r->rg_id, r->n));
    RC(upload(ctx, al, &T.rflags, r->rflags, r->n));
    RC(upload(ctx, al, &T.qn_off, r->qn_off, r->n));
    RC(upload(ctx, al, &T.qn_len, r->qn_len, r->n));
    RC(upload(ctx, al, &T.qn_blob, r->qn_blob, (int64_t)r->qn_blob_bytes + 16));
// ... 225 lines not shown
}

namespace {

int read_bam_pass(cc_ctx* ctx, int32_t gid) {
    Group& g = *ctx->groups[gid];
    const DevTable& T = ctx->tables[g.table];
    const int64_t S = g.S;
    int brc = 0;
    int32_t* d_srec = (int32_t*)g.buf["stream_rec"].p;
    int32_t* d_sreg = (int32_t*)g.buf["stream_region"].p;
    int32_t* d_run = (int32_t*)g.buf["region_run"].p;
    uint32_t* d_nresid = plan_slot(ctx, g, "n_resid", &brc);
    uint32_t* d_nbig = plan_slot(ctx, g, "n_big", &brc);
    uint32_t* d_ndrop = plan_slot(ctx, g, "n_drop", &brc);
    if (brc) return brc;
    const bool coord = g.coord_sorted && S > 0;
    const bool coord_pair = coord && !g.force_sort;
    const bool members = g.badread != 0;
    g.members_built = false;
    uint32_t* n_long = plan_slot(ctx, g, "n_long", &brc);
    if (brc) return brc;
    uint64_t lsize = 1 << 10;
    {
        const uint64_t want = g.fast && g.plan.count("n_long") ? (uint64_t)(2 * g.plan["n_long"]) + (uint64_t)S / 16
                                                               : (uint64_t)S;
        while (lsize < want) lsize <<= 1;
    }
    unsigned long long* ltab = nullptr;
    const char* lpm = getenv("CC_LP_MIN");
    const int64_t lp_min = lpm ? atoll(lpm) : LP_MIN;
    const bool lpart = coord_pair && !getenv("CC_LTAB_CAS") &&
                       (lp_min == 0 || (g.fast && g.plan.count("n_long") && g.plan.count("scan_pairs") &&
                                        g.plan["n_long"] >= lp_min));
    if (coord_pair && !lpart && !getenv("CC_LTAB_OFF")) ltab = GB(unsigned long long, "pc_ltab", (int64_t)lsize);
    uint64_t* pkeys = nullptr;
    uint32_t* pcount = nullptr;
    uint32_t pcap = 0;
    if (lpart) {
        pcap = (uint32_t)std::min<int64_t>((g.fast && g.plan.count("scan_pairs") ? g.plan["scan_pairs"] : S / 2) + 4096,
                                           INT32_MAX);
        pkeys = GB(uint64_t, "pc_pkeys", pcap);
        pcount = plan_slot(ctx, g, "lp_found", &brc);
        if (brc) return brc;
    }
    Fills fill(ctx);
    RC(fill.add(ctx->d_err, 4, 0u));
    RC(fill.add(ctx->d_cnt, sizeof(unsigned long long) * CC_NUM_COUNTERS * CNT_STRIPES, 0u));
    RC(fill.add(g.buf["plan_totals"].p, 4 * PLAN_SLOTS, 0u));
    if (g.buf.count("plan_stripes") && g.buf["plan_stripes"].p)
        RC(fill.add(g.buf["plan_stripes"].p, sizeof(uint32_t) * PLAN_SLOTS * PSTRIPES * PSTRIDE, 0u));
    g.stripes_pending = false;
    if (ltab) RC(fill.add(ltab, sizeof(unsigned long long) * lsize, ~0u));
    bool drop_zeroed = false;
    if (g.fast && g.plan.count("scan_fam") && g.plan["scan_fam"] > 0) {
        int32_t* fd = GB(int32_t, "fam_drop", g.plan["scan_fam"]);
        RC(fill.add(fd, sizeof(int32_t) * g.plan["scan_fam"], 0u));
        drop_zeroed = true;
    }
    bool pre_ends = false, pre_csn = false;
    if (g.fast && g.plan.count("scan_pairs") && g.plan.count("scan_fam")) {
        const int64_t Rp = 2 * g.plan["scan_pairs"], Fp = g.plan["scan_fam"];
        const bool deep_planned = !g.coord_sorted || Rp == 0 || g.plan.count("n_big");
        if (Rp > 0 && deep_planned) {
            uint8_t* cf = GB(uint8_t, "cflag", (Rp + 15) & ~15LL);
            RC(fill.add(cf, ((size_t)Rp + 15) & ~(size_t)15, 0u));
            pre_ends = true;
        }
        if (Fp > 0 && deep_planned) {
            const int64_t nd = g.coord_sorted && Rp > 0 ? g.plan["n_big"] : 0;
            const bool tiles = g.coord_sorted && g.ident && Rp > 0;
            uint64_t size = 1024;
            while (size < (uint64_t)(tiles ? 2 * std::min(nd, Fp) : 2 * Fp)) size <<= 1;
            unsigned long long* ht = GB(unsigned long long, "csn_ht_key", (int64_t)size);
            RC(fill.add(ht, sizeof(unsigned long long) * size, ~0u));
            pre_csn = true;
        }
    }
    uint64_t* rq = nullptr;
    int32_t* spos = nullptr;
    if (coord_pair && !g.ident) {
        rq = GB(uint64_t, "pc_rq", T.n);
        spos = GB(int32_t, "pc_spos", T.n);
        RC(fill.add(rq, sizeof(uint64_t) * T.n, ~0u));
        RC(fill.add(spos, sizeof(int32_t) * T.n, ~0u));
    }
    int32_t* pre = nullptr;
    if (g.coord_sorted && T.n > 0) { pre = GB(int32_t, "rec_e", T.n); }
    uint32_t* d_ndg = T.ndeep;
    const int64_t dcap = 0;
    int32_t* dlist = nullptr;
    if (g.coord_sorted && T.n > 0) dlist = T.dlist;
    uint64_t* skey = GB(uint64_t, "skey", S);
    uint32_t* sval = GB(uint32_t, "sval", S);
    uint64_t* skey2 = GB(uint64_t, "skey2", S);
    uint32_t* sval2 = GB(uint32_t, "sval2", S);
    uint8_t* badflag = GB(uint8_t, "badflag", (S + 15) & ~15LL);
    int32_t* mate_of = GB(int32_t, "mate_of", S);
    uint8_t* pflag = GB(uint8_t, "pflag", (S + 15) & ~15LL);
    const int64_t N = T.n;
    int32_t* partner = nullptr;
    int32_t* claims = nullptr;
    if (coord_pair) {
        partner = GB(int32_t, "pc_partner", S);
        claims = GB(int32_t, "pc_claims", S);
    }
// ... 40 lines not shown
    }
    const int64_t NDG = dlist ? T.n_deep : 0;
    g.n_deepg = NDG;
    uint32_t* deep_gid = nullptr;
    bool deep_q = false;
    uint32_t* d_nmulti = plan_slot(ctx, g, "n_multi", &brc);
    if (brc) return brc;
    bool sorted_pairing = false;
    uint64_t* rk_app = nullptr;
    uint32_t* rv_app = nullptr;
    uint32_t* n_app = nullptr;
    if (coord) {
        uint64_t* rkey = T.rkey;
        int32_t* rec_e = GB(int32_t, "rec_e", N);
        if (coord_pair) {
            uint8_t* resid = GB(uint8_t, "pc_resid", (S + 15) & ~15LL);
            if (!g.ident) {
                ProfScope ps(ctx, "k_pair_coord");
                hipLaunchKernelGGL(k_scatter_stream, dim3(nblk(S)), dim3(256), 0, ctx->stream, S, g.ident, d_srec, skey, spos, rq);
            }
            const uint64_t* qk = g.ident ? (const uint64_t*)skey : (const uint64_t*)rq;
            uint64_t* gq = nullptr;
            int32_t* gend = nullptr;
            uint32_t* boff = nullptr;
            unsigned long long* dgk = nullptr;
            uint64_t dgsize = 64;
            if (NDG > 0) {
                while (dgsize < (uint64_t)(2 * NDG)) dgsize <<= 1;
                gq = GB(uint64_t, "deep_gq", N);
                gend = GB(int32_t, "deep_gend", N);
                boff = GB(uint32_t, "deep_boff", N + 1);
                const bool ranked_plan = g.fast && g.plan.count("deep_ovf") && g.plan["deep_ovf"] == 0 &&
                                         !g.no_deep_fam && !getenv("CC_DEEP_SORT");
                if (!ranked_plan) deep_gid = GB(uint32_t, "deep_gid", N);
                deep_q = true;
                dgk = GB(unsigned long long, "deep_dgk", 2 * (int64_t)dgsize);
                RC(fill.add(dgk, sizeof(unsigned long long) * 2 * dgsize, 0xFFFFFFFEu));
                RC(fill.launch());
                ProfScope pq(ctx, "k_deep_qsort");
                hipLaunchKernelGGL(k_deep_qsort, dim3((unsigned)std::min<int64_t>(NDG, CC_DQ_GRID)), dim3(DQ_T), 0, ctx->stream,
                                   (const uint32_t*)d_ndg, (const int32_t*)dlist, N, (const uint64_t*)rkey, qk, gq, gend,
                                   boff, dgk, dgsize - 1, deep_gid);
            }
            uint32_t* lst = plan_stripes(ctx, g, n_long, &brc);
            if (brc) return brc;
            ProfScope ps(ctx, "k_pair_coord");
            const char* pct = getenv("CC_PC_TILE");
            const bool small = pct ? atoi(pct) == 512 : N < PC_SMALL_N;
            if (small)
                hipLaunchKernelGGL(k_pair_coord_tile<512>, dim3(nblk(N, 512)), dim3(256), 0, ctx->stream, N, qk,
                                   g.ident ? (const int32_t*)nullptr : (const int32_t*)spos, rkey, T, partner, claims,
                                   mate_of, pflag, ltab, lsize - 1, lst, ctx->d_err, (const uint64_t*)gq,
                                   (const int32_t*)gend, (const uint32_t*)boff, (const unsigned long long*)dgk,
                                   dgsize - 1, pkeys, pcount, pcap);
            else
                hipLaunchKernelGGL(k_pair_coord_tile<1024>, dim3(nblk(N, 1024)), dim3(256), 0, ctx->stream, N, qk,
                                   g.ident ? (const int32_t*)nullptr : (const int32_t*)spos, rkey, T, partner, claims,
                                   mate_of, pflag, ltab, lsize - 1, lst, ctx->d_err, (const uint64_t*)gq,
                                   (const int32_t*)gend, (const uint32_t*)boff, (const unsigned long long*)dgk,
                                   dgsize - 1, pkeys, pcount, pcap);
            hipLaunchKernelGGL(k_stripe_total, dim3(1), dim3(64), 0, ctx->stream, lst, n_long);
            uint32_t* st = plan_stripes(ctx, g, d_nresid, &brc);
            if (brc) return brc;
            rk_app = GB(uint64_t, "pc_rk_app", S);
            rv_app = GB(uint32_t, "pc_rv_app", S);
            n_app = plan_slot(ctx, g, "resid_app", &brc);
            if (brc) return brc;
            hipLaunchKernelGGL(k_pair_resid, dim3((unsigned)((S + PD_TILE - 1) / PD_TILE)), dim3(256), 0, ctx->stream, S,
                               skey, partner, claims, resid, st, ltab, lsize - 1, n_long, ctx->d_err, rk_app, rv_app, n_app);
            if (g.fast && g.plan.count("n_resid")) g.stripes_pending = true;
            else hipLaunchKernelGGL(k_stripe_total, dim3(1), dim3(64), 0, ctx->stream, st, d_nresid);
        }
    }
        if (lpart) {
            uint32_t* hist = GB(uint32_t, "lp_hist", (int64_t)LP_BUCKETS * LP_NB);
            uint32_t* off = GB(uint32_t, "lp_off", (int64_t)LP_BUCKETS * LP_NB);
            uint64_t* bkeys = GB(uint64_t, "lp_bkeys", pcap);
            uint32_t* lp_tot = plan_slot(ctx, g, "lp_total", &brc);
            if (brc) return brc;
            {
                ProfScope pl(ctx, "k_lp_check");
                hipLaunchKernelGGL(k_lp_hist, dim3(LP_NB), dim3(LP_T), 0, ctx->stream, (const uint64_t*)pkeys,
                                   (const uint32_t*)pcount, pcap, hist);
            }
            RC(scan_launch<false>(ctx, (const uint32_t*)hist, (int64_t)LP_BUCKETS * LP_NB, lp_tot, "k_lp_check",
                                  ScanStore{off}));
            ProfScope pl(ctx, "k_lp_check");
            hipLaunchKernelGGL(k_lp_scatter, dim3(LP_NB), dim3(LP_T), 0, ctx->stream, (const uint64_t*)pkeys,
                               (const uint32_t*)pcount, pcap, (const uint32_t*)off, bkeys);
            hipLaunchKernelGGL(k_lp_dups, dim3(LP_BUCKETS), dim3(LP_T), 0, ctx->stream, (const uint32_t*)pcount, pcap,
                               (const uint32_t*)off, (const uint64_t*)bkeys, ctx->d_err);
        }
    if (coord_pair) {
        int64_t NL = 0;
        RC(planned_total(ctx, g, "n_long", n_long, &NL));
        const uint8_t* resid = (const uint8_t*)g.buf["pc_resid"].p;
        int64_t NR = 0;
        RC(planned_total(ctx, g, "n_resid", d_nresid, &NR));
        if (NR > 0) {
            const bool many = NR > S / 4;
            uint64_t hsize = 1024, bsize = 1024;
            while (!many && hsize < (uint64_t)(2 * NR)) hsize <<= 1;
            while (!many && bsize < (uint64_t)(NR / 4 + 1)) bsize <<= 1;
            unsigned long long* rht = nullptr;
            unsigned long long* bloom = nullptr;
            uint32_t *hcnt = nullptr, *hmin = nullptr, *hmax = nullptr;
            uint32_t* d_rmulti = plan_slot(ctx, g, "resid_multi", &brc);
            if (brc) return brc;
            if (!many) {
                rht = GB(unsigned long long, "pc_rht", (int64_t)hsize);
                bloom = GB(unsigned long long, "pc_bloom", (int64_t)bsize);
                hcnt = GB(uint32_t, "pc_hcnt", (int64_t)hsize);
                hmin = GB(uint32_t, "pc_hmin", (int64_t)hsize);
                hmax = GB(uint32_t, "pc_hmax", (int64_t)hsize);
                RC(fill.add(rht, sizeof(unsigned long long) * hsize, ~0u));
                RC(fill.add(bloom, sizeof(unsigned long long) * bsize, 0u));
                RC(fill.add(hcnt, sizeof(uint32_t) * hsize, 0u));
                RC(fill.add(hmin, sizeof(uint32_t) * hsize, ~0u));
                RC(fill.add(hmax, sizeof(uint32_t) * hsize, 0u));
                RC(fill.launch());
            }
            uint64_t* rk = GB(uint64_t, "pc_rk", NR);
            uint32_t* rv = GB(uint32_t, "pc_rv", NR);
            int64_t NR2 = 0;
            const bool appended = !many && rk_app && !getenv("CC_RESID_SCAN");
            if (appended) {
                ProfScope ps(ctx, "k_pair_resid");
                hipLaunchKernelGGL(k_resid_insert, dim3(nblk(NR)), dim3(256), 0, ctx->stream, (const uint32_t*)n_app, NR,
                                   (const uint64_t*)rk_app, (const uint32_t*)rv_app, rht, hsize - 1, bloom, bsize - 1,
                                   hcnt, hmin, hmax, d_rmulti, ctx->d_err);
            } else {
                RC(scan_emit(ctx, g, resid, S, &NR2, "scan_resid",
                             EmitResid{skey, rk, rv, NR, rht, hsize - 1, bloom, bsize - 1, ctx->d_err, hcnt, hmin, hmax,
                                       d_rmulti}));
            }
            if (!many) {
                ProfScope ps(ctx, "k_pair_resid");
                hipLaunchKernelGGL(k_resid_probe, dim3(nblk(S)), dim3(256), 0, ctx->stream, S, skey, resid,
                                   (const unsigned long long*)rht, hsize - 1, (const unsigned long long*)bloom, bsize - 1,
                                   ctx->d_err);
            }
            int64_t nmulti_r = 1;
            if (!many) RC(planned_total(ctx, g, "resid_multi", d_rmulti, &nmulti_r));
            if (!many && nmulti_r == 0 && !getenv("CC_RESID_SORT")) {
                ProfScope ps(ctx, "k_pair_mark");
                hipLaunchKernelGGL(k_resid_pair, dim3(nblk(NR)), dim3(256), 0, ctx->stream, NR,
                                   (const uint64_t*)(appended ? rk_app : rk), (const uint32_t*)(appended ? rv_app : rv),
                                   (const unsigned long long*)rht, hsize - 1, (const uint32_t*)hcnt,
                                   (const uint32_t*)hmin, (const uint32_t*)hmax, g.ident, d_srec, T, mate_of, pflag,
                                   ctx->d_err, ctx->d_cnt);
            } else {
            if (appended)
                RC(scan_emit(ctx, g, resid, S, &NR2, "scan_resid",
                             EmitResid{skey, rk, rv, NR, nullptr, 0, nullptr, 0, ctx->d_err, nullptr, nullptr, nullptr,
                                       nullptr}));
            RC(sort_pairs(ctx, rk, skey2, rv, sval2, NR, "sort_qname_resid"));
            if (many) {
                ProfScope ps(ctx, "k_pair_resid");
                hipLaunchKernelGGL(k_resid_probe_sorted, dim3(nblk(S)), dim3(256), 0, ctx->stream, S, skey, resid,
                                   (const uint64_t*)skey2, NR, ctx->d_err);
            }
            ProfScope ps(ctx, "k_pair_mark");
            uint32_t* mst = plan_stripes(ctx, g, d_nmulti, &brc);
            if (brc) return brc;
            hipLaunchKernelGGL(k_pair_mark, dim3(nblk(NR)), dim3(256), 0, ctx->stream, NR, skey2, sval2, g.ident, d_srec, T,
                               mate_of, pflag, ctx->d_err, ctx->d_cnt, mst);
            sorted_pairing = true;
            hipLaunchKernelGGL(k_stripe_total, dim3(1), dim3(64), 0, ctx->stream, mst, d_nmulti);
            }
        }
    } else {
        RC(sort_pairs(ctx, skey, skey2, sval, sval2, S, "sort_qname"));
        if (S > 0) {
            ProfScope ps(ctx, "k_pair_mark");
            uint32_t* mst = plan_stripes(ctx, g, d_nmulti, &brc);
            if (brc) return brc;
            hipLaunchKernelGGL(k_pair_mark, dim3(nblk(S)), dim3(256), 0, ctx->stream, S, skey2, sval2, g.ident, d_srec, T,
                               mate_of, pflag, ctx->d_err, ctx->d_cnt, mst);
            sorted_pairing = true;
            hipLaunchKernelGGL(k_stripe_total, dim3(1), dim3(64), 0, ctx->stream, mst, d_nmulti);
        }
    }
    int64_t P = 0;
    int32_t* pr_rec1 = GB(int32_t, "pr_rec1", S);
    int32_t* pr_rec2 = GB(int32_t, "pr_rec2", S);
    int32_t* pr_region = GB(int32_t, "pr_region", S);
    RC(scan_emit(ctx, g, pflag, S, &P, "scan_pairs",
                 EmitPairs{mate_of, g.ident, d_srec, d_sreg, pr_rec1, pr_rec2, pr_region,
                           g.coord_sorted ? (int32_t*)g.buf["rec_e"].p : nullptr}));
    g.P = P;
    pr_rec1 = GB(int32_t, "pr_rec1", P);
    pr_rec2 = GB(int32_t, "pr_rec2", P);
    pr_region = GB(int32_t, "pr_region", P);
    int4* pr_tag = GB(int4, "pr_tag", P);
    const PairView PV{pr_rec1, pr_rec2, pr_region, d_run, g.scoped, pr_tag};
    const int64_t R = 2 * P;
    g.R = R;
    uint64_t* chash = GB(uint64_t, "chash", P);
    uint64_t* thash = nullptr, *rhash = nullptr;
    int4* rtag = nullptr;
    if (g.coord_sorted) {
        rhash = GB(uint64_t, "rec_thash", N);
        const auto nb = g.plan.find("n_big");
        const bool by_rec = nb != g.plan.end() ? nb->second * 8 <= R : NDG == 0;
        if (by_rec && !getenv("CC_GR_BY_PAIR")) rtag = GB(int4, "rec_tag", N);
    }
    else { thash = GB(uint64_t, "thash", R); }
    uint32_t* tval = g.coord_sorted ? nullptr : GB(uint32_t, "tval", R);
    uint64_t* rs_key = GB(uint64_t, "rs_key", R);
    uint32_t* rs_val = GB(uint32_t, "rs_val", R);
    uint8_t* cflag = GB(uint8_t, "cflag", (R + 15) & ~15LL);
    uint32_t* bigE = nullptr;
    if (g.coord_sorted && R > 0) {
        bigE = GB(uint32_t, "grp_bigE", R);
    }
    if (R > 0 && !pre_ends) RC(fill.add(cflag, ((size_t)R + 15) & ~(size_t)15, 0u));
    RC(fill.launch());
    if (P > 0) {
        ProfScope ps(ctx, "k_pair_keys");
        hipLaunchKernelGGL(k_pair_keys, dim3(nblk(P)), dim3(256), 0, ctx->stream, P, PV, T, g.seed, chash, thash,
                           tval, pr_tag, rhash, (uint2*)bigE, rtag);
    }
    g.local_groups = false;
    int32_t* mem_rec = GB(int32_t, "mem_rec", R);
    int64_t n_known = 0;
    int64_t n_deep = 0;
    bool deep_same_group = false;
    bool deep_ranked = false;
    if (g.coord_sorted && R > 0) {
        int32_t* rec_e = (int32_t*)g.buf["rec_e"].p;
        const uint64_t* rkey = (const uint64_t*)T.rkey;
        const int64_t NT = (N + GT - 1) / GT;
        uint32_t* tsmall = GB(uint32_t, "grp_tile_small", NT);
        {
            ProfScope ps(ctx, "k_group");
            uint32_t* st = plan_stripes(ctx, g, d_nbig, &brc);
            if (brc) return brc;
            if (getenv("CC_GROUP_STAGED"))
                hipLaunchKernelGGL(k_group_flags, dim3(nblk(N, GT)), dim3(GT), 0, ctx->stream, N, rkey, rec_e, tsmall, st);
            else
                hipLaunchKernelGGL(k_group_count, dim3(nblk(N, GT * GC_TILES)), dim3(GT), 0, ctx->stream, N, (const int32_t*)rec_e,
                                   (const uint8_t*)T.rdeep, tsmall, st);
            if (g.fast && g.plan.count("n_big")) g.stripes_pending = true;
            else hipLaunchKernelGGL(k_stripe_total, dim3(1), dim3(64), 0, ctx->stream, st, d_nbig);
        }
        int64_t NS = 0, NB = 0;
        uint32_t* tpre = GB(uint32_t, "grp_tile_pre", NT);
        RC(scan_total(ctx, g, tsmall, tpre, NT, &NS, "scan_small"));
        if (NS > 0) {
            ProfScope ps(ctx, "k_group_rank");
            uint8_t* segf0 = GB(uint8_t, "segf", (R + 15) & ~15LL);
            uint32_t* valid0 = GB(uint32_t, "mem_valid", R);
            uint4* meta0 = nullptr;
            if (members) { meta0 = GB(uint4, "mem_meta", R); }
            if (rtag)
                hipLaunchKernelGGL(k_group_rank<true>, dim3(nblk(N, GT)), dim3(GT), 0, ctx->stream, N, rkey, rec_e,
                                   (const uint64_t*)rhash, (const uint32_t*)tpre, rs_key, rs_val, mem_rec, PV,
                                   (const int4*)rtag, T, segf0, valid0, meta0, ctx->d_err);
            else
                hipLaunchKernelGGL(k_group_rank<false>, dim3(nblk(N, GT)), dim3(GT), 0, ctx->stream, N, rkey, rec_e,
                                   (const uint64_t*)rhash, (const uint32_t*)tpre, rs_key, rs_val, mem_rec, PV,
                                   (const int4*)nullptr, T, segf0, valid0, meta0, ctx->d_err);
        }
        n_known = NS;
        RC(planned_total(ctx, g, "n_big", d_nbig, &NB));
        n_deep = NB;
        if (NS + NB != R) {
            uint32_t eb = 0;
            RC(read_err(ctx, &eb));
            if (eb & EB_NEEDSORT) return CC_E_NEEDSORT;
            ctx->err = "position-group partition lost read ends";
            return CC_E_INVALID;
        }
        g.local_groups = NB == 0;
        if (NB > 0 && deep_q && NDG > 0 && !g.no_deep_fam && !getenv("CC_DEEP_SORT")) {
            const int32_t* gend = (const int32_t*)g.buf["deep_gend"].p;
            uint32_t* gcnt = GB(uint32_t, "deep_gcnt", NDG);
            uint32_t* goff = GB(uint32_t, "deep_goff", NDG);
            uint32_t* se = GB(uint32_t, "deep_se", N);
            int4* items = GB(int4, "deep_items", NB);
            int4* bigit = GB(int4, "deep_big", NB / 65 + 1);
            uint32_t* d_ovf = plan_slot(ctx, g, "deep_ovf", &brc);
            if (brc) return brc;
            uint32_t* d_items = plan_slot(ctx, g, "deep_items", &brc);
            if (brc) return brc;
            uint32_t* d_big = plan_slot(ctx, g, "deep_big", &brc);
            if (brc) return brc;
            uint8_t* segf1 = GB(uint8_t, "segf", (R + 15) & ~15LL);
            uint32_t* valid1 = GB(uint32_t, "mem_valid", R);
            uint4* meta1 = nullptr;
            if (members) { meta1 = GB(uint4, "mem_meta", R); }
            const DeepOut dout{R, rs_val, mem_rec, segf1, valid1, meta1};
            {
                ProfScope ps(ctx, "k_deep_count");
                hipLaunchKernelGGL(k_deep_count, dim3((unsigned)std::min<int64_t>(NDG, 4096)), dim3(256), 0, ctx->stream,
                                   (const uint32_t*)d_ndg, (const int32_t*)dlist, gend, (const int32_t*)rec_e, gcnt);
            }
            int64_t nd = 0;
            RC(scan_total(ctx, g, gcnt, goff, NDG, &nd, "scan_deep"));
            if (nd != NB) {
                ctx->err = "deep position groups: end count differs from the group partition";
                return CC_E_INVALID;
            }
            {
                ProfScope ps(ctx, "k_deep_fam");
                hipLaunchKernelGGL(k_deep_fam, dim3((unsigned)std::min<int64_t>(NDG, CC_DF_GRID)), dim3(DF_T), 0, ctx->stream,
                                   (const uint32_t*)d_ndg, (const int32_t*)dlist, gend, (const int32_t*)rec_e,
                                   (const uint64_t*)rhash, (const uint32_t*)goff, NS, PV, T, se, items, d_items, bigit,
                                   d_big, d_ovf, ctx->d_err);
            }
#ifdef DF_PROF
            {
                unsigned long long hp[8];
                HIPCHK(hipStreamSynchronize(ctx->stream));
                HIPCHK(hipMemcpyFromSymbol(hp, HIP_SYMBOL(g_df_prof), sizeof(hp)));
// ... 11 lines not shown
                    hipLaunchKernelGGL(k_deep_emit, dim3((unsigned)std::min<int64_t>(NB / 256 + 1, 8192)), dim3(256), 0,
                                       ctx->stream, (const int4*)items, (const uint32_t*)d_items, (const uint32_t*)se, PV,
                                       T, dout, ctx->d_err);
                }
                int64_t nbig = 0;
                RC(planned_total(ctx, g, "deep_big", d_big, &nbig));
                if (nbig > 0) {
                    ProfScope ps(ctx, "k_deep_sortfam");
                    hipLaunchKernelGGL(k_deep_sortfam, dim3((unsigned)std::min<int64_t>(nbig, CC_DS_GRID)), dim3(DF_ST), 0,
                                       ctx->stream, (const int4*)bigit, (const uint32_t*)d_big, (const uint32_t*)se, PV, T,
                                       dout, ctx->d_err);
                }
                deep_ranked = true;
            }
        }
        if (NB > 0 && !deep_ranked) {
            uint32_t* bx = GB(uint32_t, "grp_bx", R);
            RC(scan_total(ctx, g, bigE, bx, R, &NB, "scan_bigE"));
            uint64_t* bkey = GB(uint64_t, "grp_bkey", NB);
            uint32_t* bval = GB(uint32_t, "grp_bval", NB);
            int gbits = 1;
            while ((1LL << gbits) < NDG) ++gbits;
            const char* kbe = getenv("CC_DEEP_KEYBITS");
            const int kb = kbe ? atoi(kbe) : 48;
            const bool by_group = deep_gid != nullptr && kb > 0 && gbits <= 24;
            deep_same_group = by_group;
            hipLaunchKernelGGL(k_big_keys, dim3(nblk(R)), dim3(256), 0, ctx->stream, R, bigE, bx,
                               (const uint64_t*)rhash, PV, (const uint32_t*)(by_group ? deep_gid : nullptr), gbits,
                               by_group ? kb : 64, bkey, bval);
            RC(sort_pairs(ctx, bkey, rs_key + NS, bval, rs_val + NS, NB, "sort_tags_big", 0u, by_group ? (unsigned)kb : 64u));
        }
    } else {
        RC(sort_pairs(ctx, thash, rs_key, tval, rs_val, R, "sort_tags"));
    }
    uint8_t* segf = GB(uint8_t, "segf", (R + 15) & ~15LL);
    uint32_t* validf = GB(uint32_t, "mem_valid", R);
    uint4* mem_meta = nullptr;
    if (members) { mem_meta = GB(uint4, "mem_meta", R); }
    if (R > 0) {
        ProfScope ps(ctx, "k_fam_mark");
        if (R > n_known && !deep_ranked)
            hipLaunchKernelGGL(k_fam_mark, dim3(nblk(R - n_known)), dim3(256), 0, ctx->stream, R, n_known, n_known, rs_key,
                               rs_val, PV, T, segf, validf, mem_rec, mem_meta, ctx->d_err, deep_same_group ? 1 : 0);
        if (sorted_pairing)
        hipLaunchKernelGGL(k_fam_dedup, dim3(std::min<unsigned>(nblk(R), 1024u)), dim3(256), 0, ctx->stream, R,
                           (const uint32_t*)d_nmulti, (const uint8_t*)segf, validf, (const int32_t*)mem_rec,
                           (const uint32_t*)rs_val, (const int32_t*)pr_rec1, (const uint64_t*)T.rdig, mem_meta);
    }
    int64_t F = 0, V = 0;
    const int64_t Fcap = g.fast && g.plan.count("scan_fam") ? g.plan["scan_fam"] : R;
    int32_t* fam_beg = GB(int32_t, "fam_beg", Fcap);
    int32_t* fam_drop = GB(int32_t, "fam_drop", Fcap);
    if (Fcap > 0 && !drop_zeroed) HIPCHK(hipMemsetAsync(fam_drop, 0, sizeof(int32_t) * Fcap, ctx->stream));
    RC(scan_emit(ctx, g, segf, R, &F, "scan_fam", EmitFamStarts{validf, fam_beg, fam_drop, d_ndrop, Fcap, ctx->d_err}));
    g.F = F;
    fam_beg = GB(int32_t, "fam_beg", F);
    int32_t* fam_end = GB(int32_t, "fam_end", F);
    int32_t* fam_n = GB(int32_t, "fam_n", F);
    int32_t* fam_first = GB(int32_t, "fam_first", F);
    int32_t* fam_region = GB(int32_t, "fam_region", F);
    uint64_t* fam_hash = GB(uint64_t, "fam_hash", F);
    int32_t* cfam = GB(int32_t, "cfam", R);
    int32_t* fam_o = GB(int32_t, "fam_o", F);
    g.fam_tags_built = false;
    TagKey* fam_tag = nullptr;
    int32_t* fam_rec = nullptr;
    if (!g.badread) {
        fam_tag = GB(TagKey, "fam_tag", F);
        fam_rec = GB(int32_t, "fam_rec", F);
    }
    if (F > 0) {
        ProfScope ps(ctx, "k_fam_build");
        hipLaunchKernelGGL(k_fam_build, dim3(nblk(F)), dim3(256), 0, ctx->stream, F, R, n_known,
                           (int)(g.n_regions == 1), fam_beg, fam_drop,
                           rs_val, rs_key, pr_region, (const uint64_t*)(g.coord_sorted ? g.buf["rec_thash"].p : nullptr),
                           (const int32_t*)mem_rec, fam_end, fam_n, fam_first, fam_region, fam_hash, cflag,
                           cfam, fam_o, PV, T, fam_tag, fam_rec);
    }
    g.fam_tags_built = fam_tag != nullptr;
    RC(planned_total(ctx, g, "n_drop", d_ndrop, &V));
    V = R - V;
    int64_t F2 = 0;
    int32_t* fam_by_k = GB(int32_t, "fam_by_k", F);
    int32_t* fam_k = GB(int32_t, "fam_k", F);
    int32_t* pair_by_k = GB(int32_t, "pair_by_k", F);
    int32_t* fsz = GB(int32_t, "fam_sizes_by_creation", F);
    RC(scan_emit(ctx, g, cflag, R, &F2, "scan_creation", EmitCreation{cfam, fam_n, fam_by_k, fam_k, pair_by_k, fsz}));
    uint32_t* csegf = GB(uint32_t, "csegf", F);
    uint8_t* emark = GB(uint8_t, "emark", (F + 15) & ~15LL);
    int32_t* e1k = GB(int32_t, "e1k", F);
    bool fast_ok = false;
    if (F > 0) {
        const bool tiles = g.coord_sorted && g.ident && bigE;
        uint64_t size = 1024;
        while (size < (uint64_t)(tiles ? 2 * std::min<int64_t>(n_deep, F) : 2 * F)) size <<= 1;
        unsigned long long* cht = GB(unsigned long long, "csn_ht_key", (int64_t)size);
        uint32_t* shared = plan_slot(ctx, g, "csn_shared", &brc);
        if (brc) return brc;
        if (!pre_csn) RC(fill.add(cht, sizeof(unsigned long long) * size, ~0u));
        RC(fill.launch());
        {
            ProfScope ps(ctx, "k_csn_fast");
            hipLaunchKernelGGL(k_csn_fast, dim3((unsigned)((F + CT - 1) / CT)), dim3(256), 0, ctx->stream, F, pair_by_k,
                               chash, tiles ? (const uint32_t*)bigE : (const uint32_t*)nullptr,
                               cht, size - 1, emark, e1k, shared);
        }
        int64_t sh = 0;
        RC(planned_total(ctx, g, "csn_shared", shared, &sh));
        fast_ok = sh == 0;
    }
    if (F > 0 && !fast_ok) {
        uint64_t* ekey = GB(uint64_t, "ekey", F);
        uint32_t* eval = GB(uint32_t, "eval", F);
        uint64_t* es_key = GB(uint64_t, "es_key", F);
        uint32_t* es_val = GB(uint32_t, "es_val", F);
        hipLaunchKernelGGL(k_csn_keys, dim3(nblk(F)), dim3(256), 0, ctx->stream, F, fam_by_k, fam_first, chash, ekey, eval);
        RC(sort_pairs(ctx, ekey, es_key, eval, es_val, F, "sort_csn"));
        HIPCHK(hipMemsetAsync(emark, 0, std::max<int64_t>(F, 1), ctx->stream));
        ProfScope ps(ctx, "k_csn");
        hipLaunchKernelGGL(k_csn_mark, dim3(nblk(F)), dim3(256), 0, ctx->stream, F, es_key, es_val, fam_by_k,
                           fam_first, PV, T, csegf, ctx->d_err);
        hipLaunchKernelGGL(k_csn_entries, dim3(nblk(F)), dim3(256), 0, ctx->stream, F, csegf, es_val, fam_by_k,
                           fam_region, g.badread ? 0 : 1, emark, e1k, ctx->d_cnt);
    }
    g.csn_fast = fast_ok;
    int64_t E = 0;
    int32_t* ent_f = GB(int32_t, "ent_f", 2 * F);
    int32_t* ent_pair = GB(int32_t, "ent_pair", F);
    uint8_t* has2 = GB(uint8_t, "has2", (F + 15) & ~15LL);
    RC(scan_emit(ctx, g, emark, F, &E, "scan_entries",
                 EmitEntries{e1k, fam_by_k, pair_by_k, ent_f, ent_pair, fam_o, has2}));
    g.E = E;
    ent_f = GB(int32_t, "ent_f", 2 * E);
    ent_pair = GB(int32_t, "ent_pair", E);
    if (g.n_regions > 1 && g.badread && E > 0)
        hipLaunchKernelGGL(k_overlap_keyerror, dim3(nblk(E)), dim3(256), 0, ctx->stream, E, (const int32_t*)ent_f,
                           (const int32_t*)fam_beg, (const int32_t*)fam_end, (const int32_t*)fam_region,
                           (const uint32_t*)rs_val, (const int32_t*)pr_region, ctx->d_err);
    uint32_t bits = 0;
    bool plan_ok = true;
    RC(finish_pass(ctx, g, &bits, true, &plan_ok));
    if (bits & EB_NEEDSORT) return CC_E_NEEDSORT;
    if (bits & EB_DEEPSORT) return CC_E_DEEPSORT;
    if (!plan_ok) return CC_E_PLAN;
    g.counters[CC_CNT_COUNTER] = S - g.counters[CC_CNT_FOREIGN] - g.counters[CC_CNT_UNMAPPED];
    g.counters[CC_CNT_PAIRS] = P;
    g.counters[CC_CNT_READ_ENDS] = R;
    g.counters[CC_CNT_FAMILIES] = F;
    g.counters[CC_CNT_ENTRIES] = E;
    g.counters[CC_CNT_DROPPED] = R - V;
    g.members_built = members;
    return err_code(ctx, bits);
}

int read_bam_run(cc_ctx* ctx, int32_t gid) {
    Group& g = *ctx->groups[gid];
    auto run = [&]() {
        int rc = run_planned(ctx, g, "read_bam", [&] { return read_bam_pass(ctx, gid); });
        for (int k = 0; k < 2 && (rc == CC_E_NEEDSORT || rc == CC_E_DEEPSORT); ++k) {
            if (rc == CC_E_NEEDSORT) g.force_sort = true;
            else g.no_deep_fam = true;
            g.planned["read_bam"] = false;
            rc = run_planned(ctx, g, "read_bam", [&] { return read_bam_pass(ctx, gid); });
        }
        return rc;
    };
    int rc = run();
    if (rc == CC_E_COLLISION && !ctx->full_qhash.count(g.table)) {
        ctx->full_qhash.insert(g.table);
        g.planned["read_bam"] = false;
        rc = run();
    }
    return rc;
}

}

extern "C" {

int cc_read_bam(cc_ctx* ctx, int32_t table_id, int64_t S, const int32_t* stream_rec, const int32_t* stream_region,
                int32_t n_regions, const int32_t* region_run, const cc_read_bam_params* prm, int32_t* group_id) {
    if (!ctx || !prm || !group_id || !ctx->tables.count(table_id) || S < 0 || S >= INT32_MAX / 2) return CC_E_INVALID;
    HIPCHK(hipSetDevice(ctx->device));
    int32_t gid = ctx->next_id++;
// ... 1298 lines not shown
```

consensuscruncher_amd/engine.py:

```python
import ctypes as C
import os

import numpy as np

from . import native as N
from .consensus_helper import region_list, region_runs

MODE_SSCS, MODE_DUPLEX = 0, 1


class Interner(object):
    def __init__(self):
        self.h = N.io().ccio_interner_new()

    def __del__(self):
        try:
            if self.h:
                N.io().ccio_interner_free(self.h)
        except Exception:
            pass

    def size(self, kind):
        return int(N.io().ccio_interner_size(self.h, kind))

# ... 412 lines not shown
        dec = np.zeros(max(n, 1), np.int32)
        part = np.zeros(max(n, 1), np.int64)
        seq = qual = meta = None
        ta, ra, tx, rx, stride = -1, None, -1, None, 0
        if vote is not None:
            ta, ra, tx, rx = vote
            ra = np.ascontiguousarray(ra, np.int32)
            rx = np.ascontiguousarray(rx if rx is not None else np.zeros(0, np.int32), np.int32)
            ml = max(self.tables[ta].max_len, self.tables[tx].max_len if tx >= 0 else 0)
            stride = (ml + 15) & ~15
            seq = np.zeros((max(n, 1), stride // 2), np.uint8)
            qual = np.zeros((max(n, 1), stride), np.uint8)
            meta = np.zeros((max(n, 1), 5), np.int32)
        self._check(self.lib.cc_duplex_join(self.h, int(mode), n, N.ptr(k), N.ptr(p), m, N.ptr(x), k.shape[1],
                                            N.ptr(dec), N.ptr(part), ta, N.ptr(ra), tx, N.ptr(rx), N.ptr(seq),
                                            N.ptr(qual), N.ptr(meta), stride))
        if vote is None:
            return dec[:n], part[:n]
        return dec[:n], part[:n], (unpack_nibbles(seq[:n], stride), qual[:n], meta[:n])

    def comm_init(self, world, rank, uid):
        c = N.P()
        self._check(self.lib.cc_comm_init(self.h, int(world), int(rank), uid, C.byref(c)))
        return c

    def reduce_stats(self, comm, counters, fam_count=None, fam_first=None):
        fl = 0 if fam_count is None else len(fam_count)
        self._check(self.lib.cc_reduce_stats(self.h, comm, N.ptr(counters), len(counters),
                                             N.ptr(fam_count) if fl else None, N.ptr(fam_first) if fl else None, fl))

    def allreduce_max(self, comm, v):
        self._check(self.lib.cc_allreduce_max(self.h, comm, N.ptr(v), len(v)))

    def set_profiling(self, on):
        self._check(self.lib.cc_set_profiling(self.h, int(on)))

    def profile_only(self, names=()):
        self._check(self.lib.cc_profile_only(self.h, "\n".join(names).encode()))

    def launch_count(self):
        return int(self.lib.cc_launch_count())

    def kernel_times(self):
        names = C.create_string_buffer(1 << 16)
        ms = np.zeros(256, np.float64)
        cnt = np.zeros(256, np.int64)
        k = self.lib.cc_kernel_times(self.h, names, 1 << 16, N.ptr(ms), N.ptr(cnt), 256)
        nm = names.value.decode().split("\n")[:k]
        return {nm[i]: (float(ms[i]), int(cnt[i])) for i in range(k)}

    def synchronize(self):
        self._check(self.lib.cc_synchronize(self.h))

    def deferred(self, calls):
        self._check(self.lib.cc_defer(self.h, 1))
        try:
            calls()
        finally:
            self.lib.cc_defer(self.h, 0)
            rc = self.lib.cc_commit(self.h)
        if rc == N.CC_E_REPLAY:
            calls()
        else:
            self._check(rc)


def comm_unique_id():
    buf = C.create_string_buffer(128)
    rc = N.amd().cc_comm_unique_id(buf, 128)
    if rc != 0:
        raise N.CCError(rc, "RCCL unique id")
    return buf.raw


def duplex_tag(tag):
    t = tag.encode()
    buf = C.create_string_buffer(2 * len(t) + 16)
    k = N.io().ccio_duplex_tag(t, buf, len(buf))
    if k < 0:
        raise IndexError(N.io_error())
    return buf.value.decode()


def pack_keys(tags, width=None):
    raw = [t.encode() for t in tags]
    w = width or max([len(r) for r in raw] + [1])
    w = (w + 3) & ~3
    out = np.zeros((len(raw), w), np.uint8)
    for i, r in enumerate(raw):
        if len(r) > w:
            raise ValueError("tag longer than the key width")
        out[i, :len(r)] = np.frombuffer(r, np.uint8)
    return out


def unpack_nibbles(packed, stride):
    out = np.zeros((packed.shape[0], stride), np.uint8)
    out[:, 0::2] = packed >> 4
    out[:, 1::2] = packed & 15
    return out


def csn_names(interner, ckey9, suffix):
    n = len(suffix)
    off = np.zeros(n + 1, np.int64)
    ck = np.ascontiguousarray(ckey9, np.int32)
# ... 219 lines not shown
```

consensuscruncher_amd/native.py:

```python
import ctypes as C
import os

import numpy as np

LIBDIR = os.path.join(os.path.dirname(os.path.abspath(__file__)), "lib")

CC_E = {
    -1: "CC_E_INVALID", -2: "CC_E_HIP", -3: "CC_E_N_HIGHQ", -4: "CC_E_BAD_BASE", -5: "CC_E_SHORT_READ",
    -6: "CC_E_NO_QUAL", -7: "CC_E_NO_CIGAR", -8: "CC_E_DUP_QNAME", -9: "CC_E_AMBIGUOUS",
    -10: "CC_E_COLLISION", -11: "CC_E_UNSUPPORTED", -12: "CC_E_KEYERROR",
    -13: "CC_E_REPLAY",
}
CC_E_N_HIGHQ = -3
CC_E_COLLISION = -10
CC_E_KEYERROR = -12
CC_E_REPLAY = -13

CNT = dict(COUNTER=0, UNMAPPED=1, UNMAPPED_MATE=2, MULTIPLE_MAPPING=3, BAD_SPACER=4, PAIRS=5, READ_ENDS=6,
           FAMILIES=7, ENTRIES=8, UNPAIRED=9, ORPHAN_TAGS=10, DROPPED=11, BAD_LISTED=12, FOREIGN=13)
NUM_COUNTERS = 16
REGION_MOVED = 1 << 30

OUT_RAW, OUT_RENAME, OUT_NEW = 0, 1, 2
W_SORT, W_INDEX, W_ASYNC, W_MEMORY = 1, 2, 4, 8
# ... 74 lines not shown
    "ccio_merge_bams": (C.c_int, [C.c_char_p, P, C.c_int, C.c_int, C.c_int]),
    "ccio_write_bam_ex": (C.c_int, [C.c_char_p, P, P, C.c_int64, P, P, C.c_int, P, P, P, P, C.c_int, C.c_int, C.c_int,
                                    C.POINTER(P)]),
    "ccio_sort_bam_ex": (C.c_int, [C.c_char_p, C.c_char_p, C.c_int, C.c_int, C.c_int]),
    "ccio_merge_handles": (C.c_int, [C.c_char_p, P, C.c_int, C.c_int, C.c_int, C.c_int, C.POINTER(P)]),
    "ccio_concat_bams": (C.c_int, [C.c_char_p, P, C.c_int, C.c_int, C.c_int]),
    "ccio_index_bam": (C.c_int, [C.c_char_p]),
    "ccio_extract_barcodes": (C.c_int, [C.c_char_p, C.c_char_p, C.c_char_p, C.c_char_p, P, C.c_int32, C.c_int, P, P,
                                        P, P]),
    "ccio_fq_open": (P, [C.c_char_p, C.c_char_p, C.c_int32, C.c_int]),
    "ccio_fq_close": (None, [P]),
    "ccio_fq_info": (C.c_int, [P, i64p, i32p]),
    "ccio_fq_heads": (C.c_int, [P, C.c_int32, P, P, P, P]),
    "ccio_fq_write": (C.c_int, [P, C.c_char_p, C.c_int, P, P, C.c_int32, P, P, P, P, P, C.c_int32, C.c_int]),
    "ccio_bam_open_regions": (P, [C.c_char_p, C.c_int32, P, P, P, C.c_int]),
    "ccio_bam_cores": (C.c_int, [P, P, P, P, P, P]),
    "ccio_bam_pack": (C.c_int64, [P, C.c_int64, P, P, C.c_int64]),
    "ccio_bam_combine": (P, [P, P, C.c_int32, P, P, C.c_int32, C.c_int, C.c_int]),
    "ccio_bam_origin": (C.c_int, [P, P]),
    "ccio_bam_write_all": (C.c_int, [C.c_char_p, P, C.c_int, C.c_int]),
    "ccio_bam_write_ex": (C.c_int, [C.c_char_p, P, C.c_int, C.c_int, C.c_int]),
    "ccio_bam_route": (P, [P, P, C.c_int32, P, P, C.c_int32, C.c_int, C.c_int]),
    "ccio_bam_is_sorted": (C.c_int, [P, C.c_int]),
    "ccio_region_stream": (C.c_int64, [C.c_int64, P, P, C.c_int32, C.c_int32, P, P, P, P, P]),
    "ccio_stream_sent": (C.c_int, [C.c_int64, P, P, P, P, P, P, C.c_int32, P, P, P, C.c_int32, P, P, C.c_int32, P, P]),
    "ccio_bai_mapped": (C.c_int64, [C.c_char_p]),
    "ccio_bai_region_bytes": (C.c_int, [C.c_char_p, C.c_int32, P, P, P, P]),
    "ccio_write_columns": (C.c_int, [C.c_char_p, C.c_char_p, C.c_int32, P, P, C.c_int64, P, P, P, P, P, P, P, P,
                                     P, P, P, P, C.c_int32, P, P, P, P, C.c_int, C.c_int]),
}

AMD_SIGS = {
    "cc_create": (C.c_int, [C.c_int, C.POINTER(P)]),
    "cc_destroy": (C.c_int, [P]),
    "cc_last_error": (C.c_char_p, [P]),
    "cc_host_alloc": (P, [P, C.c_uint64]),
    "cc_host_free": (None, [P, P]),
    "cc_set_profiling": (C.c_int, [P, C.c_int]),
    "cc_profile_only": (C.c_int, [P, C.c_char_p]),
    "cc_kernel_times": (C.c_int, [P, C.c_char_p, C.c_int, P, P, C.c_int]),
    "cc_synchronize": (C.c_int, [P]),
    "cc_bgzf_deflate": (C.c_int64, [P, P, C.c_uint64, P, C.c_uint64, P, C.c_int64]),
    "cc_bgzf_hook": (C.c_int, [P, C.POINTER(P), C.POINTER(P)]),
    "cc_defer": (C.c_int, [P, C.c_int]),
    "cc_commit": (C.c_int, [P]),
    "cc_debug_skew_plan": (C.c_int, [P, C.c_int32, C.c_char_p, C.c_int64]),
    "cc_debug_build": (C.c_int, []),
    "cc_launch_count": (C.c_int64, []),
    "cc_table_upload": (C.c_int, [P, C.POINTER(cc_records), C.c_int32, i32p]),
    "cc_table_free": (C.c_int, [P, C.c_int32]),
    "cc_table_derive": (C.c_int, [P, C.c_int32]),
    "cc_table_fetch": (C.c_int64, [P, C.c_int32, C.c_char_p, P, C.c_int64]),
    "cc_guard_reruns": (C.c_int64, [P]),
    "cc_debug_poison": (C.c_int, [P, C.c_int32, C.c_char_p, C.c_int64, C.c_int32]),
    "cc_read_bam": (C.c_int, [P, C.c_int32, C.c_int64, P, P, C.c_int32, P, C.POINTER(cc_read_bam_params), i32p]),
    "cc_read_bam_rerun": (C.c_int, [P, C.c_int32, C.c_uint64]),
    "cc_group_counters": (C.c_int, [P, C.c_int32, P]),
    "cc_group_free": (C.c_int, [P, C.c_int32]),
    "cc_consensus_maker": (C.c_int, [P, C.c_int32, C.c_double, i64p]),
    "cc_duplex_consensus": (C.c_int, [P, C.c_int32, P, C.c_int32, i64p]),
    "cc_singleton_correction": (C.c_int, [P, C.c_int32, C.c_int32, P, C.c_int32, i64p]),
    "cc_fetch": (C.c_int64, [P, C.c_int32, C.c_char_p, P, C.c_int64]),
    "cc_sscs_vote": (C.c_int, [P, C.c_int32, P, P, C.c_int64, C.c_double, P, P, P, C.c_int32]),
    "cc_pair_vote": (C.c_int, [P, C.c_int32, C.c_int32, C.c_int32, P, P, C.c_int64, P, P, P, C.c_int32]),
    "cc_group": (C.c_int, [P, C.c_int64, P, C.c_int32, P, P, i64p]),
    "cc_duplex_join": (C.c_int, [P, C.c_int32, C.c_int64, P, P, C.c_int64, P, C.c_int32, P, P, C.c_int32, P,
                                 C.c_int32, P, P, P, P, C.c_int32]),
    "cc_extract_barcodes": (C.c_int, [P, C.c_int64, P, P, P, P, C.c_char_p, P, C.c_int32, P, P, P, P, P, P, P, P, P]),
    "cc_comm_unique_id": (C.c_int, [C.c_char_p, C.c_int32]),
    "cc_comm_init": (C.c_int, [P, C.c_int32, C.c_int32, C.c_char_p, C.POINTER(P)]),
    "cc_comm_destroy": (C.c_int, [P]),
    "cc_reduce_stats": (C.c_int, [P, P, P, C.c_int32, P, P, C.c_int32]),
    "cc_allreduce_max": (C.c_int, [P, P, P, C.c_int32]),
}


def _bind(lib, sigs):
    for name, (res, args) in sigs.items():
        fn = getattr(lib, name)
        fn.restype = res
        fn.argtypes = args
    return lib


def io():
    global _io
    if _io is None:
        path = os.path.join(LIBDIR, "libccio.so")
        if not os.path.exists(path):
            raise ImportError("libccio.so not built; run __graft_entry__.build()")
        _io = _bind(C.CDLL(path), IO_SIGS)
    return _io


def amd_path():
    return os.environ.get("CCAMD_LIB") or os.path.join(LIBDIR, "libccamd.so")


def lib_sha(path=None):
    import hashlib
    h = hashlib.sha256()
    with open(path or amd_path(), "rb") as f:
        for blk in iter(lambda: f.read(1 << 20), b""):
            h.update(blk)
    return h.hexdigest()[:16]

# ... 18 lines not shown
```

include/consensuscruncher_amd.h:

```cpp
#ifndef CONSENSUSCRUNCHER_AMD_H
#define CONSENSUSCRUNCHER_AMD_H

#include <stdint.h>

#ifdef __cplusplus
extern "C" {
#endif

#define CC_OK 0
#define CC_E_INVALID -1
#define CC_E_HIP -2
#define CC_E_N_HIGHQ -3
#define CC_E_BAD_BASE -4
#define CC_E_SHORT_READ -5
#define CC_E_NO_QUAL -6
#define CC_E_NO_CIGAR -7
#define CC_E_DUP_QNAME -8
#define CC_E_AMBIGUOUS -9
#define CC_E_COLLISION -10
#define CC_E_UNSUPPORTED -11
#define CC_E_KEYERROR -12
#define CC_E_REPLAY -13

#define CC_RF_BAD_SPACER 1u
// ... 127 lines not shown
                       const int32_t *ref_lens, int64_t n, const int32_t *tid, const int32_t *pos,
                       const int32_t *mtid, const int32_t *mpos, const int32_t *tlen, const uint16_t *flag,
                       const uint8_t *mapq, const uint8_t *qn_blob, const int64_t *qn_off, const int32_t *cig_id,
                       const uint32_t *cig_ops, const int64_t *cig_off, int32_t read_len, const uint8_t *seq_ascii,
                       const uint8_t *qual, const int32_t *rg_id, const char *const *rg_vals, int level,
                       int nthreads);

typedef struct cc_ctx cc_ctx;

enum {
    CC_CNT_COUNTER = 0,
    CC_CNT_UNMAPPED,
    CC_CNT_UNMAPPED_MATE,
    CC_CNT_MULTIPLE_MAPPING,
    CC_CNT_BAD_SPACER,
    CC_CNT_PAIRS,
    CC_CNT_READ_ENDS,
    CC_CNT_FAMILIES,
    CC_CNT_ENTRIES,
    CC_CNT_UNPAIRED,
    CC_CNT_ORPHAN_TAGS,
    CC_CNT_DROPPED,
    CC_CNT_BAD_LISTED,
    CC_CNT_FOREIGN,
    CC_NUM_COUNTERS = 16
};

typedef struct cc_read_bam_params {
    int32_t delim_filter;
    int32_t badread_file;
    int32_t scope_by_run;
    int32_t coord_sorted;
    uint64_t seed;
} cc_read_bam_params;

int cc_create(int device_id, cc_ctx **ctx);
int cc_destroy(cc_ctx *ctx);
const char *cc_last_error(cc_ctx *ctx);
void *cc_host_alloc(cc_ctx *ctx, uint64_t bytes);
void cc_host_free(cc_ctx *ctx, void *p);
int cc_set_profiling(cc_ctx *ctx, int on);
int cc_profile_only(cc_ctx *ctx, const char *names);
int cc_kernel_times(cc_ctx *ctx, char *names, int names_cap, double *ms, int64_t *launches, int cap);
int cc_synchronize(cc_ctx *ctx);
int64_t cc_bgzf_deflate(cc_ctx *ctx, const uint8_t *data, uint64_t n, uint8_t *stage, uint64_t slot,
                        uint32_t *out_len, int64_t cap);
int cc_bgzf_hook(cc_ctx *ctx, ccio_deflate_fn *fn, void **user);
int cc_defer(cc_ctx *ctx, int on);
int cc_commit(cc_ctx *ctx);
int cc_debug_skew_plan(cc_ctx *ctx, int32_t group_id, const char *name, int64_t delta);
int cc_debug_build(void);
int64_t cc_launch_count(void);
int64_t cc_guard_reruns(cc_ctx *ctx);
int cc_debug_poison(cc_ctx *ctx, int32_t group_id, const char *name, int64_t bytes, int32_t value);

int cc_table_upload(cc_ctx *ctx, const cc_records *rec, int32_t max_len, int32_t *table_id);
int cc_table_free(cc_ctx *ctx, int32_t table_id);
int cc_table_derive(cc_ctx *ctx, int32_t table_id);
int64_t cc_table_fetch(cc_ctx *ctx, int32_t table_id, const char *name, void *dst, int64_t cap);

#define CC_REGION_MOVED (1 << 30)
int cc_read_bam(cc_ctx *ctx, int32_t table_id, int64_t n_stream, const int32_t *stream_rec,
                const int32_t *stream_region, int32_t n_regions, const int32_t *region_run,
                const cc_read_bam_params *params, int32_t *group_id);
int cc_group_counters(cc_ctx *ctx, int32_t group_id, int64_t *counters );
int cc_group_free(cc_ctx *ctx, int32_t group_id);

int cc_consensus_maker(cc_ctx *ctx, int32_t group_id, double cutoff, int64_t *n_out);
int cc_read_bam_rerun(cc_ctx *ctx, int32_t group_id, uint64_t seed);
int cc_duplex_consensus(cc_ctx *ctx, int32_t group_id, const int32_t *bc_swap, int32_t n_bc, int64_t *n_out);
int cc_singleton_correction(cc_ctx *ctx, int32_t singleton_group, int32_t sscs_group, const int32_t *bc_swap,
                            int32_t n_bc, int64_t *n_out);

int64_t cc_fetch(cc_ctx *ctx, int32_t group_id, const char *name, void *dst, int64_t cap);


int cc_sscs_vote(cc_ctx *ctx, int32_t table_id, const int32_t *member_index, const int64_t *fam_offsets,
                 int64_t nfam, double cutoff, uint8_t *out_seq_nib, uint8_t *out_qual, int32_t *out_meta,
                 int32_t out_stride);
int cc_pair_vote(cc_ctx *ctx, int32_t mode, int32_t table_a, int32_t table_b, const int32_t *rec_a,
                 const int32_t *rec_b, int64_t n, uint8_t *out_seq_nib, uint8_t *out_qual, int32_t *out_meta,
                 int32_t out_stride);

int cc_group(cc_ctx *ctx, int64_t n, const void *keys, int32_t key_bytes, int32_t *out_perm,
             int64_t *out_fam_offsets, int64_t *out_nfam);
int cc_duplex_join(cc_ctx *ctx, int32_t mode, int64_t n, const void *keys, const void *partner_keys, int64_t m,
                   const void *x_keys, int32_t key_bytes, int32_t *out_decision, int64_t *out_partner,
                   int32_t table_a, const int32_t *rec_a, int32_t table_x, const int32_t *rec_x,
                   uint8_t *out_seq_nib, uint8_t *out_qual, int32_t *out_meta, int32_t out_stride);

int cc_extract_barcodes(cc_ctx *ctx, int64_t n, const uint8_t *h1, const uint8_t *h2, const int32_t *len1,
                        const int32_t *len2, const char *pattern, const char *const *blist, int32_t nblist,
                        uint8_t *out_status, char *out_bc, int32_t *out_cut1, int32_t *out_cut2, uint32_t *out_bad1,
                        uint32_t *out_bad2, int64_t *counts, int64_t *r1_hist, int64_t *r2_hist);

typedef struct cc_comm cc_comm;
int cc_comm_unique_id(char *id, int32_t cap );
int cc_comm_init(cc_ctx *ctx, int32_t world, int32_t rank, const char *id, cc_comm **comm);
int cc_comm_destroy(cc_comm *comm);
int cc_reduce_stats(cc_ctx *ctx, cc_comm *comm, int64_t *counters, int32_t n_counters, int64_t *fam_count,
                    int64_t *fam_first, int32_t fam_len);
int cc_allreduce_max(cc_ctx *ctx, cc_comm *comm, int64_t *v, int32_t n);


#ifdef __cplusplus
}
// ... 3 lines not shown
```

Baseline: 2.977 billion.

## Produce scan tile counts in producer kernels to skip scan up-sweep pass

Producer kernels (pair coordination, residual pairing, group rank, family creation, csn_fast) now count flagged elements per scan tile with wave ballots and atomics. This lets the following scans use these partial counts directly instead of running a separate upsweep/count pass. The down-sweep checks its count against the tile total and sets an error bit, with a rerun fallback on mismatch. The cost is extra atomics and shared-memory reductions inside the producers, plus more complex correctness conditions.

```diff
diff --git a/consensuscruncher_amd/csrc/cc_engine.hip b/consensuscruncher_amd/csrc/cc_engine.hip
--- a/consensuscruncher_amd/csrc/cc_engine.hip
+++ b/consensuscruncher_amd/csrc/cc_engine.hip
@@ -49,6 +49,7 @@
     EB_PLAN = 1u << 11,
     EB_DEEPSORT = 1u << 15,
     EB_SCANWAIT = 1u << 16,
+    EB_SCANCOUNT = 1u << 18,
     EB_GUARD = 1u << 17,
 };
 
@@ -495,6 +496,39 @@
 #pragma unroll
     for (int o = 32; o > 0; o >>= 1) v += __shfl_xor(v, o);
     if (t == 0) *total = v;
+}
+
+constexpr int SCAN_T = 256, SCAN_I = 16, SCAN_TILE = SCAN_T * SCAN_I;
+struct ScanCnt {
+    uint32_t* part;
+    uint32_t nb;
+};
+__device__ __forceinline__ void scan_count(const ScanCnt& c, int64_t i, bool f) {
+    if (!c.part) return;
+    const uint32_t tile = (uint32_t)(i / SCAN_TILE);
+    const int lane = threadIdx.x & 63;
+    f = f && i >= 0 && tile < c.nb;
+    uint64_t m = __ballot(f);
+    while (m) {
+        const int ld = __ffsll((unsigned long long)m) - 1;
+        const uint32_t tl = (uint32_t)__shfl((int)tile, ld, 64);
+        const uint64_t same = __ballot(f && tile == tl);
+        if (lane == ld) atomicAdd(c.part + tl, (uint32_t)__popcll(same));
+        m &= ~same;
+    }
+}
+__device__ __forceinline__ void scan_count_block(const ScanCnt& c, int64_t tile, uint32_t v, uint32_t* s_red) {
+    if (!c.part) return;
+#pragma unroll
+    for (int o = 32; o > 0; o >>= 1) v += __shfl_xor(v, o, 64);
+    if ((threadIdx.x & 63) == 0) s_red[threadIdx.x >> 6] = v;
+    __syncthreads();
+    if (threadIdx.x == 0) {
+        uint32_t t = 0;
+        for (int w = 0; w < (int)(blockDim.x >> 6); ++w) t += s_red[w];
+        if ((t & 0xffffu) && tile >= 0 && tile < c.nb) atomicAdd(c.part + tile, t & 0xffffu);
+        if ((t >> 16) && tile + 1 >= 0 && tile + 1 < c.nb) atomicAdd(c.part + tile + 1, t >> 16);
+    }
 }
 
 struct FillSet {
@@ -969,13 +1003,14 @@
                                             int32_t* __restrict__ claimer, int32_t* __restrict__ mate_of,
                                             uint8_t* __restrict__ pflag, unsigned long long* __restrict__ ltab,
                                             uint64_t lmask, uint32_t& n_long, bool both_search,
-                                            uint32_t* __restrict__ err) {
+                                            uint32_t* __restrict__ err, int32_t* flagged = nullptr) {
     partner[s] = sx;
     claimer[sx] = (int32_t)s;
     const int32_t s1 = (int32_t)s < sx ? (int32_t)s : sx, s2 = (int32_t)s < sx ? sx : (int32_t)s;
     mate_of[s2] = s1;
     pflag[s2] = 1;
     const bool enters = !both_search || s == s2;
+    if (flagged && enters) *flagged = s2;
     if (ltab && s2 - s1 > PD_W && enters) {
         ++n_long;
         uint64_t h = key & lmask;
@@ -1007,8 +1042,9 @@
                                                          const uint32_t* __restrict__ boff,
                                                          const unsigned long long* __restrict__ dgk, uint64_t dgmask,
                                                          uint64_t* __restrict__ pkeys, uint32_t* __restrict__ pcount,
-                                                         uint32_t pcap) {
+                                                         uint32_t pcap, ScanCnt pcnt) {
     __shared__ uint64_t s_k[(TILE + PC_HALO + GRP_SMALL + 2)], s_q[(TILE + PC_HALO + GRP_SMALL + 2)];
+    __shared__ uint32_t s_red[256 / 64];
     const int64_t t0 = xcd_block() * TILE;
     const int64_t t1 = min(N, t0 + TILE);
     const int64_t w0 = t0 > PC_HALO ? t0 - PC_HALO : 0;
@@ -1104,19 +1140,24 @@
             ok[u] = cand[u] >= 0 && d == 0;
         }
     }
-    uint32_t nl = 0, na = 0;
+    uint32_t nl = 0, na = 0, npf = 0;
     uint64_t ak[PC_PER];
 #pragma unroll
     for (int u = 0; u < PC_PER; ++u) {
         ak[u] = 0;
+        int32_t fl = -1;
         if (ok[u]) {
             const int32_t r = (int32_t)(t0 + threadIdx.x + 256 * u);
             const bool both = tgt[u] == rkey[r];
             const bool enters = mate_record(spos ? spos[r] : r, spos ? spos[cand[u]] : cand[u], key[u], partner,
-                                            claimer, mate_of, pflag, ltab, lmask, nl, both, err);
+                                            claimer, mate_of, pflag, ltab, lmask, nl, both, err, &fl);
             if (pkeys && enters) ak[na++] = key[u];
         }
-    }
+        if (spos) scan_count(pcnt, fl, fl >= 0);
+        else npf += fl >= 0 ? 1u : 0u;
+    }
+    static_assert(SCAN_TILE % TILE == 0, "a search tile lies in one scan tile");
+    if (!spos) scan_count_block(pcnt, t0 / SCAN_TILE, npf, s_red);
     stripe_add(nl, long_stripes);
     if (pkeys) {
         const int lane = threadIdx.x & 63;
@@ -1369,8 +1410,10 @@
                                                     const uint32_t* __restrict__ hmax, int ident,
                                                     const int32_t* __restrict__ stream_rec, DevTable T,
                                                     int32_t* __restrict__ mate_of, uint8_t* __restrict__ pflag,
-                                                    uint32_t* __restrict__ err, unsigned long long* __restrict__ cnt) {
+                                                    uint32_t* __restrict__ err, unsigned long long* __restrict__ cnt,
+                                                    ScanCnt pcnt) {
     int acc[1] = {0};
+    int64_t fl = -1;
     const int64_t x = (int64_t)blockIdx.x * blockDim.x + threadIdx.x;
     if (x < NR) {
         const uint64_t k = rk[x];
@@ -1385,6 +1428,7 @@
                 if (qname_eq(T, ident ? (int32_t)a : stream_rec[a], ident ? (int32_t)i : stream_rec[i])) {
                     mate_of[i] = (int32_t)a;
                     pflag[i] = 1;
+                    fl = (int64_t)i;
                 } else {
                     atomicOr(err, EB_COLLISION);
                 }
@@ -1393,6 +1437,7 @@
             atomicOr(err, EB_PLAN);
         }
     }
+    scan_count(pcnt, fl, fl >= 0);
     const int slots[1] = {CC_CNT_UNPAIRED};
     block_count<1>(acc, slots, cnt);
 }
@@ -1767,8 +1812,10 @@
                                                    uint64_t* __restrict__ rs_key, uint32_t* __restrict__ rs_val,
                                                    int32_t* __restrict__ rs_rec, PairView V, const int4* __restrict__ rec_tag,
                                                    DevTable T, uint8_t* __restrict__ segf, uint32_t* __restrict__ validf,
-                                                   uint4* __restrict__ mem_meta, uint32_t* __restrict__ err) {
+                                                   uint4* __restrict__ mem_meta, uint32_t* __restrict__ err,
+                                                   ScanCnt fcnt) {
     __shared__ uint64_t s_k[GS], s_h[GS];
+    __shared__ uint32_t s_red[GT / 64];
     __shared__ int32_t s_e[GS];
     __shared__ int4 s_t[BYREC ? GS : 1];
     __shared__ int2 s_m[BYREC ? GS : 1];
@@ -1806,58 +1853,64 @@
     const int lane = t & 63;
     if (lane == 0) s_c[t >> 6] = (uint32_t)__popcll(bm);
     __syncthreads();
-    if (!sm) return;
-    const int fo = BYREC ? 0 : (int)T.flag[r];
-    const int32_t omt = BYREC ? 0 : T.mtid[r], omp = BYREC ? 0 : T.mpos[r];
-    const uint4 om = mem_meta ? T.meta[CC_IDX(r, T.n, DS_MEMBER)] : make_uint4(0u, 0u, 0u, 0u);
-    uint32_t cpv = base + (uint32_t)__popcll(bm & ((1ULL << lane) - 1ULL));
-    for (int w = 0; w < (t >> 6); ++w) cpv += s_c[w];
-    const int32_t e = s_e[li];
-    const uint64_t h = s_h[li];
-    uint32_t before = 0, rank = 0;
-    int32_t pe = -1, pj = 0;
-    uint64_t ph = 0;
-    for (int j = a; j < z; ++j) {
-        const int32_t ej = s_e[j];
-        if (ej < 0) continue;
-        const uint64_t hj = s_h[j];
-        before += j < li ? 1u : 0u;
-        if (hj < h || (hj == h && ej < e)) {
-            ++rank;
-            if (pe < 0 || hj > ph || (hj == ph && ej > pe)) { pe = ej; ph = hj; pj = j; }
-        }
-    }
-    const uint32_t o = CC_IDX(cpv - before + rank, N, DS_SLOT);
-    bool start = pe < 0 || ph != h;
-    if (!start) {
-        bool same;
-        if constexpr (BYREC) {
-            const int4 x = s_t[li], y = s_t[pj];
-            const int2 mx = s_m[li], my = s_m[pj];
-            same = x.x == y.x && x.y == y.y && x.z == y.z && x.w == y.w && mx.x == my.x && mx.y == my.y;
-        } else {
-            const int32_t rp = (int32_t)(b0 - GH + pj);
-            const int4 pt = V.tag[e >> 1], pq = V.tag[pe >> 1];
-            const int fp = T.flag[rp];
-            same = pt.x == pq.x && pt.y == pq.y && pt.z == pq.z && pt.w == pq.w && omt == T.mtid[rp] &&
-                   omp == T.mpos[rp] && ((fo >> 4) & 1) == ((fp >> 4) & 1) && which_read(fo) == which_read(fp);
-        }
-        if (!same) {
-            atomicOr(err, EB_COLLISION);
-            start = true;
-        }
-    }
-    const bool valid = start || ((e >> 1) != (pe >> 1));
-    if (start) rs_key[o] = h;
-    rs_val[o] = (uint32_t)e;
-    rs_rec[o] = r;
-    segf[o] = start ? 1 : 0;
-    validf[o] = valid ? 1u : 0u;
-    if (mem_meta) {
-        uint4 m = om;
-        m.w |= (valid ? 1u : 0u) << 23;
-        mem_meta[o] = m;
-    }
+    const uint32_t ctile = (base >= (uint32_t)GRP_SMALL ? base - (uint32_t)GRP_SMALL : 0u) / SCAN_TILE;
+    uint32_t nst = 0;
+    if (sm) {
+        const int fo = BYREC ? 0 : (int)T.flag[r];
+        const int32_t omt = BYREC ? 0 : T.mtid[r], omp = BYREC ? 0 : T.mpos[r];
+        const uint4 om = mem_meta ? T.meta[CC_IDX(r, T.n, DS_MEMBER)] : make_uint4(0u, 0u, 0u, 0u);
+        uint32_t cpv = base + (uint32_t)__popcll(bm & ((1ULL << lane) - 1ULL));
+        for (int w = 0; w < (t >> 6); ++w) cpv += s_c[w];
+        const int32_t e = s_e[li];
+        const uint64_t h = s_h[li];
+        uint32_t before = 0, rank = 0;
+        int32_t pe = -1, pj = 0;
+        uint64_t ph = 0;
+        for (int j = a; j < z; ++j) {
+            const int32_t ej = s_e[j];
+            if (ej < 0) continue;
+            const uint64_t hj = s_h[j];
+            before += j < li ? 1u : 0u;
+            if (hj < h || (hj == h && ej < e)) {
+                ++rank;
+                if (pe < 0 || hj > ph || (hj == ph && ej > pe)) { pe = ej; ph = hj; pj = j; }
+            }
+        }
+        const uint32_t o = CC_IDX(cpv - before + rank, N, DS_SLOT);
+        bool start = pe < 0 || ph != h;
+        if (!start) {
+            bool same;
+            if constexpr (BYREC) {
+                const int4 x = s_t[li], y = s_t[pj];
+                const int2 mx = s_m[li], my = s_m[pj];
+                same = x.x == y.x && x.y == y.y && x.z == y.z && x.w == y.w && mx.x == my.x && mx.y == my.y;
+            } else {
+                const int32_t rp = (int32_t)(b0 - GH + pj);
+                const int4 pt = V.tag[e >> 1], pq = V.tag[pe >> 1];
+                const int fp = T.flag[rp];
+                same = pt.x == pq.x && pt.y == pq.y && pt.z == pq.z && pt.w == pq.w && omt == T.mtid[rp] &&
+                       omp == T.mpos[rp] && ((fo >> 4) & 1) == ((fp >> 4) & 1) && which_read(fo) == which_read(fp);
+            }
+            if (!same) {
+                atomicOr(err, EB_COLLISION);
+                start = true;
+            }
+        }
+        const bool valid = start || ((e >> 1) != (pe >> 1));
+        if (start) rs_key[o] = h;
+        rs_val[o] = (uint32_t)e;
+        rs_rec[o] = r;
+        segf[o] = start ? 1 : 0;
+        if (start) nst = o / SCAN_TILE == ctile ? 1u : 1u << 16;
+        validf[o] = valid ? 1u : 0u;
+        if (mem_meta) {
+            uint4 m = om;
+            m.w |= (valid ? 1u : 0u) << 23;
+            mem_meta[o] = m;
+        }
+    }
+    static_assert(GT + 2 * GRP_SMALL <= SCAN_TILE, "a block's slots span at most two scan tiles");
+    scan_count_block(fcnt, ctile, nst, s_red);
 }
 
 __global__ __launch_bounds__(256) void k_big_keys(int64_t R, const uint32_t* __restrict__ bigE,
@@ -2379,8 +2432,10 @@
                                                    int32_t* __restrict__ fam_region, uint64_t* __restrict__ fam_hash,
                                                    uint8_t* __restrict__ cflag, int32_t* __restrict__ cfam,
                                                    int32_t* __restrict__ fam_o, PairView V, DevTable T,
-                                                   TagKey* __restrict__ fam_tag, int32_t* __restrict__ fam_rec) {
+                                                   TagKey* __restrict__ fam_tag, int32_t* __restrict__ fam_rec,
+                                                   ScanCnt ccnt) {
     int64_t f = (int64_t)blockIdx.x * blockDim.x + threadIdx.x;
+    int64_t ce = -1;
     if (f < F) {
         fam_o[f] = 0x7f7f7f7f;
         int32_t b = CC_IDX(fam_beg[f], R, DS_SLOT);
@@ -2393,6 +2448,7 @@
         fam_region[f] = one_region ? 0 : pr_region[fe >> 1];
         fam_hash[f] = rhash && b >= n_known ? rhash[CC_IDX(mem_rec[b], T.n, DS_REC)] : rs_key[b];
         cflag[fe] = 1;
+        ce = (int64_t)fe;
         cfam[fe] = (int32_t)f;
         if (fam_tag) {
             const int32_t r0 = mem_rec[b];
@@ -2400,6 +2456,7 @@
             fam_rec[f] = r0;
         }
     }
+    scan_count(ccnt, ce, ce >= 0);
 }
 
 __global__ __launch_bounds__(256) void k_fam_tags(int64_t F, const int32_t* __restrict__ fam_first,
@@ -2523,9 +2580,12 @@
                                                   const uint32_t* __restrict__ bigE,
                                                   unsigned long long* __restrict__ ht_key, uint64_t mask,
                                                   uint8_t* __restrict__ emark, int32_t* __restrict__ e1k,
-                                                  uint32_t* __restrict__ shared) {
+                                                  uint32_t* __restrict__ shared, ScanCnt ecnt) {
     __shared__ int32_t s_p[CT + CW + 2];
     __shared__ unsigned long long s_tab[CSLOTS];
+    __shared__ uint32_t s_red[256 / 64];
+    static_assert(SCAN_TILE % CT == 0, "an entry tile lies in one scan tile");
+    uint32_t nst = 0;
     const int t = threadIdx.x;
     const int64_t t0 = (int64_t)blockIdx.x * CT, t1 = min(F, t0 + CT);
     const int64_t w0 = max((int64_t)0, t0 - CW - 1), w1 = min(F, t1 + 1);
@@ -2538,6 +2598,7 @@
         const bool start = (k == 0) || s_p[k - 1 - w0] != p;
         if (k >= t0) {
             emark[k] = start ? 1 : 0;
+            nst += start ? 1u : 0u;
             if (start) e1k[k] = (k + 1 < F && s_p[k + 1 - w0] == p) ? (int32_t)(k + 1) : -1;
         }
         if (!start) continue;
@@ -2565,6 +2626,7 @@
         }
     }
     if (sh) *shared = 1u;
+    scan_count_block(ecnt, t0 / SCAN_TILE, nst, s_red);
 }
 
 
@@ -4014,7 +4076,6 @@
 }
 
 
-constexpr int SCAN_T = 256, SCAN_I = 16, SCAN_TILE = SCAN_T * SCAN_I;
 
 template <bool MAX>
 __device__ __forceinline__ uint32_t sop(uint32_t a, uint32_t b) { return MAX ? (a > b ? a : b) : a + b; }
@@ -4241,7 +4302,8 @@
 template <bool MAX, class Emit, class TIn>
 __global__ __launch_bounds__(SCAN_T) void k_scan_down(const TIn* __restrict__ in, int64_t n,
                                                       const uint32_t* __restrict__ part,
-                                                      uint32_t* __restrict__ total, Emit em) {
+                                                      uint32_t* __restrict__ total, Emit em,
+                                                      uint32_t* __restrict__ chk) {
     __shared__ uint32_t s_tile[SCAN_TILE];
     __shared__ uint32_t s_w[SCAN_T / 64];
     __shared__ uint32_t s_pre[SCAN_T / 64];
@@ -4279,6 +4341,7 @@
     uint32_t all;
     uint32_t run = sop<MAX>(pre, block_scan_excl<MAX>(t, s_w, &all));
     if (blockIdx.x == gridDim.x - 1 && tid == 0) *total = sop<MAX>(pre, all);
+    if (chk && tid == 0 && all != part[blockIdx.x]) atomicOr(chk, EB_SCANCOUNT);
 #pragma unroll
     for (int k = 0; k < SCAN_I; ++k) {
         const uint32_t x = v[k];
@@ -4654,6 +4717,7 @@
 constexpr int CC_E_PLAN = -100;
 constexpr int CC_E_NEEDSORT = -101;
 constexpr int CC_E_DEEPSORT = -102;
+constexpr int CC_E_SCANCOUNT = -104;
 constexpr int CC_E_SCANWAIT = -103;
 constexpr int PLAN_SLOTS = 64;
 
@@ -4679,6 +4743,10 @@
     bool scan_two = false;
     std::unordered_set<int32_t> full_qhash;
     int64_t scan_retries = 0;
+    bool scan_nocount = false;
+    int64_t scans_counted = 0;
+    int64_t scans_fallback = 0;
+    int64_t scan_count_reruns = 0;
     int64_t guard_reruns = 0;
     uint32_t* d_err = nullptr;
     unsigned long long* d_cnt = nullptr;
@@ -4817,7 +4885,8 @@
 }
 
 template <bool MAX, class Emit, class TIn>
-int scan_launch(cc_ctx* ctx, const TIn* in, int64_t n, uint32_t* d_tot, const char* name, Emit em);
+int scan_launch(cc_ctx* ctx, const TIn* in, int64_t n, uint32_t* d_tot, const char* name, Emit em,
+                const uint32_t* counted = nullptr);
 
 int sort_pairs(cc_ctx* ctx, const uint64_t* kin, uint64_t* kout, const uint32_t* vin, uint32_t* vout, int64_t n,
                const char* name, unsigned begin_bit = 0, unsigned end_bit = 64) {
@@ -4866,14 +4935,29 @@
 }
 
 constexpr int64_t SCAN_ONE_MAX = 64;
+bool scan_one(const cc_ctx* ctx, int64_t nb) {
+    const char* force = getenv("CC_SCAN1");
+    return !ctx->scan_two && (force ? force[0] == '1' : nb <= SCAN_ONE_MAX);
+}
+enum : uint32_t { SC_PAIRS = 1u, SC_FAM = 2u, SC_CREATION = 4u, SC_ENTRIES = 8u };
+bool scan_counting(const cc_ctx* ctx, int64_t n, uint32_t which = SC_PAIRS | SC_FAM | SC_CREATION | SC_ENTRIES) {
+    const char* e = getenv("CC_SCAN_COUNTED");
+    const uint32_t on = !e ? SC_FAM | SC_ENTRIES : e[0] == '0' ? 0u : SC_PAIRS | SC_FAM | SC_CREATION | SC_ENTRIES;
+    return !ctx->scan_nocount && (on & which) && n > 0 && !scan_one(ctx, (n + SCAN_TILE - 1) / SCAN_TILE);
+}
+const uint32_t* scan_counted(cc_ctx* ctx, const ScanCnt& c, bool all_counted) {
+    if (!c.part) return nullptr;
+    if (!all_counted) ++ctx->scans_fallback;
+    return all_counted ? c.part : nullptr;
+}
 template <bool MAX, class Emit, class TIn>
-int scan_launch(cc_ctx* ctx, const TIn* in, int64_t n, uint32_t* d_tot, const char* name, Emit em) {
+int scan_launch(cc_ctx* ctx, const TIn* in, int64_t n, uint32_t* d_tot, const char* name, Emit em,
+                const uint32_t* counted) {
     const int64_t nb = (n + SCAN_TILE - 1) / SCAN_TILE;
     uintptr_t al = (uintptr_t)in;
     if constexpr (Emit::kPlain) al |= (uintptr_t)em.out;
     if (al & 15u) { ctx->err = "scan operands must be 16-B aligned"; return CC_E_INVALID; }
-    const char* force = getenv("CC_SCAN1");
-    const bool one = !ctx->scan_two && (force ? force[0] == '1' : nb <= SCAN_ONE_MAX);
+    const bool one = scan_one(ctx, nb);
     if (one && nb > 0) {
         if (nb > ctx->scan_cap) {
             const int64_t cap = std::max<int64_t>(nb, 1 << 14);
@@ -4899,12 +4983,20 @@
                            d_tot, em, lb);
         return 0;
     }
+    if (counted && !MAX && nb > 0) {
+        ++ctx->scans_counted;
+        ProfScope ps(ctx, name);
+        hipLaunchKernelGGL((k_scan_down<MAX, Emit, TIn>), dim3((unsigned)nb), dim3(SCAN_T), 0, ctx->stream, in, n, counted,
+                           d_tot, em, ctx->d_err);
+        return 0;
+    }
     int rc = 0;
     uint32_t* part = (uint32_t*)tmp_storage(ctx, (size_t)nb * 4 + 64, &rc);
     if (!part) return rc;
     ProfScope ps(ctx, name);
     hipLaunchKernelGGL((k_scan_reduce<MAX, TIn>), dim3((unsigned)nb), dim3(SCAN_T), 0, ctx->stream, in, n, part);
-    hipLaunchKernelGGL((k_scan_down<MAX, Emit, TIn>), dim3((unsigned)nb), dim3(SCAN_T), 0, ctx->stream, in, n, part, d_tot, em);
+    hipLaunchKernelGGL((k_scan_down<MAX, Emit, TIn>), dim3((unsigned)nb), dim3(SCAN_T), 0, ctx->stream, in, n,
+                       (const uint32_t*)part, d_tot, em, (uint32_t*)nullptr);
     return 0;
 }
 
@@ -4987,22 +5079,23 @@
 
 template <class TIn>
 int scan_total(cc_ctx* ctx, Group& g, const TIn* in, uint32_t* out, int64_t n, int64_t* total,
-               const char* name) {
+               const char* name, const uint32_t* counted = nullptr) {
     if (n <= 0) { *total = 0; return 0; }
     int rc = 0;
     uint32_t* d_tot = plan_slot(ctx, g, name, &rc);
     if (rc) return rc;
-    RC(scan_launch<false>(ctx, in, n, d_tot, name, ScanStore{out}));
+    RC(scan_launch<false>(ctx, in, n, d_tot, name, ScanStore{out}, counted));
     return planned_total(ctx, g, name, d_tot, total);
 }
 
 template <class Emit, class TIn>
-int scan_emit(cc_ctx* ctx, Group& g, const TIn* in, int64_t n, int64_t* total, const char* name, Emit em) {
+int scan_emit(cc_ctx* ctx, Group& g, const TIn* in, int64_t n, int64_t* total, const char* name, Emit em,
+              const uint32_t* counted = nullptr) {
     if (n <= 0) { *total = 0; return 0; }
     int rc = 0;
     uint32_t* d_tot = plan_slot(ctx, g, name, &rc);
     if (rc) return rc;
-    RC(scan_launch<false>(ctx, in, n, d_tot, name, em));
+    RC(scan_launch<false>(ctx, in, n, d_tot, name, em, counted));
     return planned_total(ctx, g, name, d_tot, total);
 }
 
@@ -5085,7 +5178,15 @@
         rc = pass();
         ctx->scan_two = false;
     }
-    if (rc == CC_E_SCANWAIT) rc = CC_E_INVALID;
+    if (rc == CC_E_SCANCOUNT && !ctx->scan_nocount) {
+        ++ctx->scan_count_reruns;
+        fprintf(stderr, "[cc] %s: a counted scan partial differed from its flags, pass re-run (%lld)\n", stage,
+                (long long)ctx->scan_count_reruns);
+        ctx->scan_nocount = true;
+        g.verify.clear();
+        rc = pass();
+    }
+    if (rc == CC_E_SCANWAIT || rc == CC_E_SCANCOUNT) rc = CC_E_INVALID;
     g.planned[stage] = rc == 0;
     return rc;
 }
@@ -5101,6 +5202,7 @@
 
 int err_code(cc_ctx* ctx, uint32_t bits) {
     if (!bits) return 0;
+    if (bits & EB_SCANCOUNT) { ctx->err = "a counted scan partial differed from its flags"; return CC_E_SCANCOUNT; }
     if (bits & EB_COLLISION) { ctx->err = "64-bit key hash collision (retry with another seed)"; return CC_E_COLLISION; }
     if (bits & EB_KEYERROR) { ctx->err = "KeyError: read_dict[tag] already deleted (consensus_helper.py:490 with overlapping bed regions, or DCS_maker.py:258 with duplex keys that are not mutual)"; return CC_E_KEYERROR; }
     if (bits & EB_AMBIGUOUS) { ctx->err = "duplex keys are not mutual or span regions; reference outcome is order-dependent"; return CC_E_AMBIGUOUS; }
@@ -5113,6 +5215,7 @@
     if (bits & EB_THR) { ctx->err = "cutoff table too short"; return CC_E_INVALID; }
     if (bits & EB_CHAIN) { ctx->err = "a chain of duplex partners longer than the engine follows"; return CC_E_UNSUPPORTED; }
     if (bits & EB_SCANWAIT) { ctx->err = "scan look-back wait bound exceeded"; return CC_E_SCANWAIT; }
+
     if (bits & EB_TOO_LONG) { ctx->err = "record too long for the 16-bit length fields or payload > 64 GiB"; return CC_E_UNSUPPORTED; }
     if (bits & EB_GUARD) { ctx->err = "a guarded index was outside its array (no load was made from it)"; return CC_E_INVALID; }
     ctx->err = "unknown device error";
@@ -5425,6 +5528,14 @@
 int64_t cc_launch_count(void) { return g_launches.load(std::memory_order_relaxed); }
 
 int64_t cc_guard_reruns(cc_ctx* ctx) { return ctx ? ctx->guard_reruns : CC_E_INVALID; }
+
+int cc_scan_count_stats(cc_ctx* ctx, int64_t* out3) {
+    if (!ctx || !out3) return CC_E_INVALID;
+    out3[0] = ctx->scans_counted;
+    out3[1] = ctx->scans_fallback;
+    out3[2] = ctx->scan_count_reruns;
+    return 0;
+}
 
 }
 namespace {
@@ -5756,6 +5867,19 @@
         RC(fill.add(g.buf["plan_stripes"].p, sizeof(uint32_t) * PLAN_SLOTS * PSTRIPES * PSTRIDE, 0u));
     g.stripes_pending = false;
     if (ltab) RC(fill.add(ltab, sizeof(unsigned long long) * lsize, ~0u));
+    ScanCnt cnt_pairs{nullptr, 0}, cnt_fam{nullptr, 0}, cnt_creation{nullptr, 0}, cnt_entries{nullptr, 0};
+    const int64_t cnt_nb = (S + SCAN_TILE - 1) / SCAN_TILE + 1;
+    uint32_t* cnt_area = nullptr;
+    if (scan_counting(ctx, S)) {
+        cnt_area = GB(uint32_t, "scan_counts", 4 * cnt_nb);
+        RC(fill.add(cnt_area, sizeof(uint32_t) * 4 * cnt_nb, 0u));
+    }
+    auto cnt_of = [&](int k, int64_t n) {
+        const int64_t nb = (n + SCAN_TILE - 1) / SCAN_TILE;
+        return cnt_area && nb <= cnt_nb && scan_counting(ctx, n, 1u << k) ? ScanCnt{cnt_area + k * cnt_nb, (uint32_t)nb}
+                                                                           : ScanCnt{nullptr, 0};
+    };
+    cnt_pairs = cnt_of(0, S);
     bool drop_zeroed = false;
     if (g.fast && g.plan.count("scan_fam") && g.plan["scan_fam"] > 0) {
         int32_t* fd = GB(int32_t, "fam_drop", g.plan["scan_fam"]);
@@ -5902,13 +6026,13 @@
                                    g.ident ? (const int32_t*)nullptr : (const int32_t*)spos, rkey, T, partner, claims,
                                    mate_of, pflag, ltab, lsize - 1, lst, ctx->d_err, (const uint64_t*)gq,
                                    (const int32_t*)gend, (const uint32_t*)boff, (const unsigned long long*)dgk,
-                                   dgsize - 1, pkeys, pcount, pcap);
+                                   dgsize - 1, pkeys, pcount, pcap, cnt_pairs);
             else
                 hipLaunchKernelGGL(k_pair_coord_tile<1024>, dim3(nblk(N, 1024)), dim3(256), 0, ctx->stream, N, qk,
                                    g.ident ? (const int32_t*)nullptr : (const int32_t*)spos, rkey, T, partner, claims,
                                    mate_of, pflag, ltab, lsize - 1, lst, ctx->d_err, (const uint64_t*)gq,
                                    (const int32_t*)gend, (const uint32_t*)boff, (const unsigned long long*)dgk,
-                                   dgsize - 1, pkeys, pcount, pcap);
+                                   dgsize - 1, pkeys, pcount, pcap, cnt_pairs);
             hipLaunchKernelGGL(k_stripe_total, dim3(1), dim3(64), 0, ctx->stream, lst, n_long);
             uint32_t* st = plan_stripes(ctx, g, d_nresid, &brc);
             if (brc) return brc;
@@ -5998,7 +6122,7 @@
                                    (const uint64_t*)(appended ? rk_app : rk), (const uint32_t*)(appended ? rv_app : rv),
                                    (const unsigned long long*)rht, hsize - 1, (const uint32_t*)hcnt,
                                    (const uint32_t*)hmin, (const uint32_t*)hmax, g.ident, d_srec, T, mate_of, pflag,
-                                   ctx->d_err, ctx->d_cnt);
+                                   ctx->d_err, ctx->d_cnt, cnt_pairs);
             } else {
             if (appended)
                 RC(scan_emit(ctx, g, resid, S, &NR2, "scan_resid",
@@ -6037,7 +6161,8 @@
     int32_t* pr_region = GB(int32_t, "pr_region", S);
     RC(scan_emit(ctx, g, pflag, S, &P, "scan_pairs",
                  EmitPairs{mate_of, g.ident, d_srec, d_sreg, pr_rec1, pr_rec2, pr_region,
-                           g.coord_sorted ? (int32_t*)g.buf["rec_e"].p : nullptr}));
+                           g.coord_sorted ? (int32_t*)g.buf["rec_e"].p : nullptr},
+                 scan_counted(ctx, cnt_pairs, coord_pair && !sorted_pairing)));
     g.P = P;
     pr_rec1 = GB(int32_t, "pr_rec1", P);
     pr_rec2 = GB(int32_t, "pr_rec2", P);
@@ -6046,6 +6171,8 @@
     const PairView PV{pr_rec1, pr_rec2, pr_region, d_run, g.scoped, pr_tag};
     const int64_t R = 2 * P;
     g.R = R;
+    cnt_fam = cnt_of(1, R);
+    cnt_creation = cnt_of(2, R);
     uint64_t* chash = GB(uint64_t, "chash", P);
     uint64_t* thash = nullptr, *rhash = nullptr;
     int4* rtag = nullptr;
@@ -6106,11 +6233,11 @@
             if (rtag)
                 hipLaunchKernelGGL(k_group_rank<true>, dim3(nblk(N, GT)), dim3(GT), 0, ctx->stream, N, rkey, rec_e,
                                    (const uint64_t*)rhash, (const uint32_t*)tpre, rs_key, rs_val, mem_rec, PV,
-                                   (const int4*)rtag, T, segf0, valid0, meta0, ctx->d_err);
+                                   (const int4*)rtag, T, segf0, valid0, meta0, ctx->d_err, cnt_fam);
             else
                 hipLaunchKernelGGL(k_group_rank<false>, dim3(nblk(N, GT)), dim3(GT), 0, ctx->stream, N, rkey, rec_e,
                                    (const uint64_t*)rhash, (const uint32_t*)tpre, rs_key, rs_val, mem_rec, PV,
-                                   (const int4*)nullptr, T, segf0, valid0, meta0, ctx->d_err);
+                                   (const int4*)nullptr, T, segf0, valid0, meta0, ctx->d_err, cnt_fam);
         }
         n_known = NS;
         RC(planned_total(ctx, g, "n_big", d_nbig, &NB));
@@ -6228,8 +6355,10 @@
     int32_t* fam_beg = GB(int32_t, "fam_beg", Fcap);
     int32_t* fam_drop = GB(int32_t, "fam_drop", Fcap);
     if (Fcap > 0 && !drop_zeroed) HIPCHK(hipMemsetAsync(fam_drop, 0, sizeof(int32_t) * Fcap, ctx->stream));
-    RC(scan_emit(ctx, g, segf, R, &F, "scan_fam", EmitFamStarts{validf, fam_beg, fam_drop, d_ndrop, Fcap, ctx->d_err}));
+    RC(scan_emit(ctx, g, segf, R, &F, "scan_fam", EmitFamStarts{validf, fam_beg, fam_drop, d_ndrop, Fcap, ctx->d_err},
+                 scan_counted(ctx, cnt_fam, g.coord_sorted && R > 0 && n_known == R && !getenv("CC_GROUP_STAGED"))));
     g.F = F;
+    cnt_entries = cnt_of(3, F);
     fam_beg = GB(int32_t, "fam_beg", F);
     int32_t* fam_end = GB(int32_t, "fam_end", F);
     int32_t* fam_n = GB(int32_t, "fam_n", F);
@@ -6251,7 +6380,7 @@
                            (int)(g.n_regions == 1), fam_beg, fam_drop,
                            rs_val, rs_key, pr_region, (const uint64_t*)(g.coord_sorted ? g.buf["rec_thash"].p : nullptr),
                            (const int32_t*)mem_rec, fam_end, fam_n, fam_first, fam_region, fam_hash, cflag,
-                           cfam, fam_o, PV, T, fam_tag, fam_rec);
+                           cfam, fam_o, PV, T, fam_tag, fam_rec, cnt_creation);
     }
     g.fam_tags_built = fam_tag != nullptr;
     RC(planned_total(ctx, g, "n_drop", d_ndrop, &V));
@@ -6261,7 +6390,8 @@
     int32_t* fam_k = GB(int32_t, "fam_k", F);
     int32_t* pair_by_k = GB(int32_t, "pair_by_k", F);
     int32_t* fsz = GB(int32_t, "fam_sizes_by_creation", F);
-    RC(scan_emit(ctx, g, cflag, R, &F2, "scan_creation", EmitCreation{cfam, fam_n, fam_by_k, fam_k, pair_by_k, fsz}));
+    RC(scan_emit(ctx, g, cflag, R, &F2, "scan_creation", EmitCreation{cfam, fam_n, fam_by_k, fam_k, pair_by_k, fsz},
+                 scan_counted(ctx, cnt_creation, true)));
     uint32_t* csegf = GB(uint32_t, "csegf", F);
     uint8_t* emark = GB(uint8_t, "emark", (F + 15) & ~15LL);
     int32_t* e1k = GB(int32_t, "e1k", F);
@@ -6279,7 +6409,7 @@
             ProfScope ps(ctx, "k_csn_fast");
             hipLaunchKernelGGL(k_csn_fast, dim3((unsigned)((F + CT - 1) / CT)), dim3(256), 0, ctx->stream, F, pair_by_k,
                                chash, tiles ? (const uint32_t*)bigE : (const uint32_t*)nullptr,
-                               cht, size - 1, emark, e1k, shared);
+                               cht, size - 1, emark, e1k, shared, cnt_entries);
         }
         int64_t sh = 0;
         RC(planned_total(ctx, g, "csn_shared", shared, &sh));
@@ -6305,7 +6435,8 @@
     int32_t* ent_pair = GB(int32_t, "ent_pair", F);
     uint8_t* has2 = GB(uint8_t, "has2", (F + 15) & ~15LL);
     RC(scan_emit(ctx, g, emark, F, &E, "scan_entries",
-                 EmitEntries{e1k, fam_by_k, pair_by_k, ent_f, ent_pair, fam_o, has2}));
+                 EmitEntries{e1k, fam_by_k, pair_by_k, ent_f, ent_pair, fam_o, has2},
+                 scan_counted(ctx, cnt_entries, fast_ok)));
     g.E = E;
     ent_f = GB(int32_t, "ent_f", 2 * E);
     ent_pair = GB(int32_t, "ent_pair", E);
diff --git a/consensuscruncher_amd/engine.py b/consensuscruncher_amd/engine.py
--- a/consensuscruncher_amd/engine.py
+++ b/consensuscruncher_amd/engine.py
@@ -488,6 +488,11 @@
     def synchronize(self):
         self._check(self.lib.cc_synchronize(self.h))
 
+    def scan_count_stats(self):
+        out = np.zeros(3, np.int64)
+        self._check(self.lib.cc_scan_count_stats(self.h, N.ptr(out)))
+        return int(out[0]), int(out[1]), int(out[2])
+
     def deferred(self, calls):
         self._check(self.lib.cc_defer(self.h, 1))
         try:
diff --git a/consensuscruncher_amd/native.py b/consensuscruncher_amd/native.py
--- a/consensuscruncher_amd/native.py
+++ b/consensuscruncher_amd/native.py
@@ -150,6 +150,7 @@
     "cc_table_derive": (C.c_int, [P, C.c_int32]),
     "cc_table_fetch": (C.c_int64, [P, C.c_int32, C.c_char_p, P, C.c_int64]),
     "cc_guard_reruns": (C.c_int64, [P]),
+    "cc_scan_count_stats": (C.c_int, [P, P]),
     "cc_debug_poison": (C.c_int, [P, C.c_int32, C.c_char_p, C.c_int64, C.c_int32]),
     "cc_read_bam": (C.c_int, [P, C.c_int32, C.c_int64, P, P, C.c_int32, P, C.POINTER(cc_read_bam_params), i32p]),
     "cc_read_bam_rerun": (C.c_int, [P, C.c_int32, C.c_uint64]),
diff --git a/include/consensuscruncher_amd.h b/include/consensuscruncher_amd.h
--- a/include/consensuscruncher_amd.h
+++ b/include/consensuscruncher_amd.h
@@ -203,6 +203,7 @@
 int cc_debug_build(void);
 int64_t cc_launch_count(void);
 int64_t cc_guard_reruns(cc_ctx *ctx);
+int cc_scan_count_stats(cc_ctx *ctx, int64_t *out3);
 int cc_debug_poison(cc_ctx *ctx, int32_t group_id, const char *name, int64_t bytes, int32_t value);
 
 int cc_table_upload(cc_ctx *ctx, const cc_records *rec, int32_t max_len, int32_t *table_id);
```

Measured after the change: 2.975 billion (median of 2 runs). About the same (-0.1%).
